# WHU-USI3DV/GAGS

Hardware: AMD Instinct MI355X
Metric: feature-raster fwd+bwd views/s (higher is better)
Workload: dtype f32

## Files before the change

### gags_amd/_lib.py

```python
import ctypes
import os
import subprocess

import torch

_HERE = os.path.dirname(os.path.abspath(__file__))
CSRC = os.path.join(_HERE, "csrc")
LIB_PATH = os.path.join(CSRC, "libgags_hip.so")

_vp, _i32, _i64, _f32, _f64 = ctypes.c_void_p, ctypes.c_int, ctypes.c_int64, ctypes.c_float, ctypes.c_double

SIGNATURES = {
    "gags_abi_version": (_i32, []),
    "gags_strerror": (ctypes.c_char_p, [_i32]),
    "gags_device_count": (_i32, []),
    "gags_project_fwd": (_i32, [_i32, _vp, _vp, _vp, _vp, _vp, _i32, _i32, _f32, _f32, _f32, _f32,
                                _vp, _vp, _vp, _vp, _vp, _vp]),
    "gags_project_fwd_raw": (_i32, [_i32, _vp, _vp, _vp, _vp, _f32, _vp, _vp, _i32, _i32, _f32, _f32, _f32, _f32,
                                    _vp, _vp, _vp, _vp, _vp, _vp, _vp, _vp, _vp, _vp]),
    "gags_project_bwd_raw": (_i32, [_i32, _vp, _vp, _vp, _vp, _f32, _vp, _vp, _i32, _i32, _f32, _vp, _vp, _vp, _vp, _vp,
                                    _vp, _vp, _vp, _vp, _vp]),
    "gags_scan_scratch_bytes": (_i64, [_i32]),
    "gags_cumsum_i32": (_i32, [_i32, _vp, _vp, _vp, _vp, _i64, _vp]),
    "gags_cumsum_gather_i32": (_i32, [_i32, _vp, _vp, _vp, _vp, _vp, _i64, _vp]),
    "gags_read_i32": (_i32, [_vp, _vp, _vp]),
    "gags_depth_order_scratch_bytes": (_i64, [_i32]),
    "gags_depth_order": (_i32, [_i32, _vp, _vp, _vp, _vp, _vp, _i64, _vp]),
    "gags_tile_emit": (_i32, [_i32, _vp, _vp, _vp, _vp, _vp, _i32, _i32, _vp, _vp, _vp]),
    "gags_tile_emit_cap": (_i32, [_i32, _vp, _vp, _vp, _vp, _vp, _i32, _i32, _vp, _vp, _i64, _vp, _vp]),
    "gags_sort_scratch_bytes": (_i64, [_i64]),
    "gags_sort_pairs": (_i32, [_i64, _i32, _i32, _vp, _vp, _vp, _vp, _vp, _i64, _vp]),
    "gags_tile_offsets": (_i32, [_i64, _vp, _i32, _vp, _vp]),
    "gags_pack_isects": (_i32, [_i32, _i64, _vp, _vp, _vp, _vp, _vp, _vp, _vp, _vp]),
    "gags_raster_fwd_scratch_bytes": (_i64, [_i64, _i32, _i32]),
    "gags_raster_fwd": (_i32, [_i32, _i32, _i32, _i32, _vp, _vp, _vp, _vp, _vp, _vp, _vp, _i64, _vp, _vp, _vp, _vp,
                               _vp, _i64, _vp, _i32, _vp]),
    "gags_raster_bwd": (_i32, [_i32, _i32, _i32, _vp, _vp, _vp, _vp, _vp, _vp, _vp, _i64, _vp, _vp, _vp, _vp, _vp,
                               _vp, _vp, _vp, _vp, _i32, _vp]),
    "gags_bwd_rowmap_scratch_bytes": (_i64, [_i64]),
    "gags_bwd_rowmap_elems": (_i64, [_i64, _i32, _i32]),
    "gags_bwd_rowmap": (_i32, [_i64, _i32, _i32, _vp, _vp, _vp, _i64, _vp, _i64, _vp, _vp, _i64, _vp]),
    "gags_raster_bwd_geom_scratch_bytes": (_i64, [_i64, _i32, _i32, _i32, _i32, _i64]),
    "gags_raster_bwd_geom": (_i32, [_i32, _i32, _i32, _i32, _vp, _vp, _vp, _i64, _vp, _vp, _vp, _vp, _vp, _i64, _vp, _i64,
                                    _vp, _vp, _vp, _i64, _i32, _vp]),
    "gags_blended_mask": (_i32, [_i64, _i32, _i32, _i32, _vp, _vp, _i64, _vp, _vp]),
    "gags_bwd_staged_scratch_bytes": (_i64, [_i64, _i32, _i32]),
    "gags_raster_bwd_colors_staged": (_i32, [_i32, _i32, _i32, _i32, _vp, _i64, _vp, _vp, _vp, _i64, _vp, _i64, _vp,
                                             _i64, _vp, _i32, _i32, _i32, _vp, _vp, _vp, _vp, _vp, _vp]),
    "gags_raster_list_need": (_i32, [_i32, _i32, _i32, _vp, _vp, _i64, _vp, _i32, _vp, _vp]),
    "gags_trim_lists": (_i32, [_i32, _i32, _vp, _vp, _vp, _vp, _vp, _vp]),
    "gags_trim_last_ids": (_i32, [_i32, _i32, _vp, _vp, _vp, _vp, _vp]),
    "gags_raster_stats": (_i32, [_i32, _i32, _vp, _vp, _vp, _vp, _vp, _i64, _vp, _vp]),
    "gags_project_bwd": (_i32, [_i32, _vp, _vp, _vp, _vp, _vp, _i32, _i32, _f32, _vp, _vp, _vp, _vp, _vp,
                                _vp, _vp, _vp, _vp]),
    "gags_sh_fwd": (_i32, [_i32, _i32, _i32, _vp, _vp, _vp, _vp, _vp, _vp]),
    "gags_sh_bwd": (_i32, [_i32, _i32, _i32, _vp, _vp, _vp, _vp, _vp, _vp, _vp]),
    "gags_sh_bwd_dirs": (_i32, [_i32, _i32, _i32, _vp, _vp, _vp, _vp, _vp, _vp, _vp, _vp]),
    "gags_ed_normalize": (_i32, [_i64, _i32, _vp, _vp, _vp]),
    "gags_adam_step": (_i32, [_i64, _vp, _vp, _vp, _vp, _f64, _f64, _f64, _f64, _i32, _vp]),
    "gags_pack_rows": (_i32, [_i64, _vp, _vp, _i32, _i32, _i32, _i32, _vp, _i32, _vp]),
    "gags_unpack_rows": (_i32, [_i64, _vp, _vp, _i32, _vp, _vp, _i32, _i32, _i32, _i32, _vp]),
    "gags_compact_mask_scratch_bytes": (_i64, [_i32]),
    "gags_compact_mask": (_i32, [_i32, _vp, _i64, _vp, _vp, _vp, _i64, _vp]),
    "gags_compact_mask_pos": (_i32, [_i32, _vp, _i64, _vp, _vp, _vp, _vp, _i64, _vp]),
    "gags_dot_scratch_bytes": (_i64, []),
    "gags_dot_f32": (_i32, [_i64, _vp, _vp, _vp, _vp, _i64, _vp]),
    "gags_trained_seg": (_i32, [_i32, _i32, _vp, _vp, _vp, _vp]),
    "gags_entropy_fwd": (_i32, [_i64, _vp, _vp, _vp]),
    "gags_entropy_bwd": (_i32, [_i64, _vp, _f32, _vp, _vp]),
    "gags_entropy_bwd_dev": (_i32, [_i64, _vp, _vp, _vp, _vp]),
    "gags_segment_stats": (_i32, [_i64, _i32, _vp, _vp, _i32, _vp, _vp, _vp, _vp]),
    "gags_segment_stats_multi": (_i32, [_i64, _i32, _vp, _vp, _i32, _i32, _vp, _vp, _vp, _i32, _vp]),
    "gags_segment_stats_runs_copies": (_i32, [_i64, _i32, _i32, _i32]),
    "gags_segment_stats_runs": (_i32, [_i64, _i32, _vp, _vp, _i32, _i32, _vp, _vp, _vp, _i32, _vp]),
    "gags_segment_loss": (_i32, [_i32, _i32, _i32, _i32, _i64, _vp, _vp, _vp, _vp, _vp, _vp, _vp, _vp, _vp, _vp]),
    "gags_region_var_bwd_layout": (_i32, [_i64, _i32, _vp, _vp, _i32, _vp, _vp, _vp, _i32, _vp]),
    "gags_region_var_bwd_add": (_i32, [_i64, _i32, _vp, _vp, _i32, _vp, _vp, _vp, _vp, _vp]),
    "gags_region_var_bwd": (_i32, [_i64, _i32, _vp, _vp, _i32, _vp, _vp, _vp, _vp]),
    "gags_gather_seg_coef": (_i32, [_i64, _vp, _i32, _vp, _vp, _vp]),
    "gags_sam_clip_feature": (_i32, [_i32, _i32, _i32, _i32, _i32, _i32, _vp, _vp, _vp, _vp, _vp, _vp]),
    "gags_sam_clip_feature_bwd_scale": (_i32, [_i32, _i32, _i32, _i32, _i32, _i32, _vp, _vp, _vp, _vp, _vp]),
    "gags_distill_l1_map_fwd": (_i32, [_i32, _i32, _i32, _i32, _i32, _i32, _vp, _vp, _vp, _vp, _vp, _vp, _i32, _vp]),
    "gags_distill_l1_map_bwd": (_i32, [_i32, _i32, _i32, _i32, _i32, _i32, _vp, _vp, _vp, _vp, _vp, _vp, _vp, _i32, _vp]),
    "gags_decoder_head_distill_fwd": (_i32, [_i32, _i32, _i32, _i32, _i32, _i32, _i32, _vp, _vp, _vp, _vp, _vp, _vp, _vp]),
    "gags_decoder_head_distill_bwd": (_i32, [_i32, _i32, _i32, _i32, _i32, _i32, _i32, _vp, _vp, _vp, _vp, _vp, _vp, _vp, _vp]),
    "gags_decoder_head_distill_bwd_f32": (_i32, [_i32, _i32, _i32, _i32, _i32, _i32, _i32, _vp, _vp, _vp, _vp, _vp, _vp, _vp, _vp]),
    "gags_decoder_pack_input": (_i32, [_i64, _i32, _i32, _vp, _vp, _vp]),
    "gags_decoder_pack_layer": (_i32, [_i32, _i32, _vp, _vp, _vp, _vp, _vp, _vp, _vp, _vp]),
    "gags_decoder_pack_layers": (_i32, [_i32, _vp, _vp, _vp, _vp, _vp, _vp, _vp, _vp, _vp, _vp]),
    "gags_decoder_layer": (_i32, [_i64, _i32, _i32, _vp, _vp, _vp, _vp, _i32, _vp, _vp, _vp, _vp, _vp, _vp]),
    "gags_decoder_wgrad_scratch_bytes": (_i64, [_i64, _i32, _i32]),
    "gags_decoder_wgrad": (_i32, [_i64, _i32, _i32, _vp, _vp, _vp, _vp, _vp, _vp, _i64, _vp]),
    "gags_decoder_wgrad_out": (_i32, [_i64, _i32, _i32, _vp, _vp, _vp, _vp, _vp, _i32, _i32, _vp, _vp, _i64, _vp]),
    "gags_decoder_head_bwd": (_i32, [_i64, _i32, _i32, _i32, _vp, _vp, _vp, _i32, _vp]),
    "gags_decoder_unpack_grad": (_i32, [_i64, _i32, _i32, _vp, _vp, _vp]),
    "gags_decoder_head": (_i32, [_i64, _i32, _i32, _i32, _vp, _vp, _i32, _vp]),
    "gags_decoder_fwd_fused": (_i32, [_i64, _i32, _i32, _vp, _vp, _vp, _vp, _vp, _vp, _vp]),
    "gags_decoder_bwd_fused": (_i32, [_i64, _i32, _i32, _vp, _vp, _vp, _vp, _vp, _vp]),
    "gags_decoder_bwd_fused_scaled": (_i32, [_i64, _i32, _i32, _vp, _vp, _vp, _vp, _vp, _vp, _vp]),
    "gags_scale_decoder_fwd_fused": (_i32, [_i64, _i32, _vp, _vp, _vp, _vp, _vp, _vp, _vp]),
    "gags_scale_decoder_fwd_fused_head": (_i32, [_i64, _i32, _vp, _vp, _vp, _vp, _vp, _vp, _vp, _vp]),
    "gags_softmax_head_bwd_y": (_i32, [_i64, _i32, _i32, _vp, _vp, _vp, _vp]),
    "gags_scale_decoder_bwd_fused": (_i32, [_i64, _vp, _vp, _vp, _vp, _vp]),
    "gags_decoder_layer_exact": (_i32, [_i64, _i32, _i32, _vp, _vp, _i32, _vp, _vp, _i32, _vp, _vp, _vp, _vp, _i32, _vp]),
    "gags_decoder_layer_split": (_i32, [_i64, _i32, _i32, _vp, _vp, _i32, _vp, _vp, _i32, _vp, _vp, _vp, _vp, _i32, _i32, _vp]),
    "gags_decoder_wgrad_split": (_i32, [_i64, _i32, _i32, _vp, _i32, _vp, _vp, _i32, _vp, _vp, _vp, _i64, _i32, _vp]),
    "gags_decoder_wgrad_exact_scratch_bytes": (_i64, [_i64, _i32, _i32]),
    "gags_decoder_wgrad_exact": (_i32, [_i64, _i32, _i32, _vp, _i32, _vp, _vp, _i32, _vp, _vp, _vp, _i64, _vp]),
    "gags_decoder_head_bwd_exact": (_i32, [_i64, _i32, _i32, _i32, _vp, _vp, _i32, _vp, _i32, _vp]),
    **{name + "_h16": None for name in ("gags_decoder_pack_layer", "gags_decoder_pack_layers", "gags_decoder_pack_input", "gags_decoder_layer", "gags_decoder_head",
                                        "gags_decoder_wgrad_scratch_bytes", "gags_decoder_wgrad", "gags_decoder_wgrad_out",
                                        "gags_decoder_head_bwd",
                                        "gags_decoder_unpack_grad", "gags_decoder_fwd_fused", "gags_decoder_bwd_fused", "gags_decoder_bwd_fused_scaled",
                                        "gags_scale_decoder_fwd_fused", "gags_scale_decoder_bwd_fused", "gags_scale_decoder_fwd_fused_head",
                                        "gags_softmax_head_bwd_y")},
    "gags_pow2_scale": (_i32, [_vp, _f32, _f32, _vp, _vp]),
    "gags_decoder_head_distill_bwd_h16": (_i32, [_i32, _i32, _i32, _i32, _i32, _i32, _i32, _vp, _vp, _vp, _vp, _vp, _vp, _vp, _vp, _vp]),
    "gags_relevancy": (_i32, [_i64, _i32, _i32, _i32, _vp, _vp, _vp, _vp, _vp]),
    "gags_relevancy_activate_scratch_bytes": (_i64, [_i32, _i32, _i32]),
    "gags_relevancy_activate": (_i32, [_i32, _i32, _i32, _vp, _f32, _i32, _i32, _vp, _vp, _vp, _vp, _vp, _vp, _vp, _i64, _vp]),
    "gags_point_relevancy_mask_scratch_bytes": (_i64, [_i32, _i64]),
    "gags_point_relevancy_mask": (_i32, [_i32, _i64, _vp, _f32, _vp, _vp, _vp, _i64, _vp]),
    "gags_point_mask_smooth_scratch_bytes": (_i64, [_i32, _i64]),
    "gags_point_mask_smooth": (_i32, [_i32, _i64, _vp, _vp, _f64, _i32, _vp, _vp, _vp, _i64, _vp]),
    "gags_depthsample_scratch_bytes": (_i64, [_i64, _i32, _i32, _i32]),
    "gags_depthsample_map": (_i32, [_i64, _i32, _i32, _i32, _vp, _vp, _vp, _vp, _f32, _i32, _vp, _vp, _vp, _vp, _i64, _vp]),
    "gags_depthsample_scatter": (_i32, [_i64, _i32, _i32, _i32, _vp, _vp, _vp, _vp, _f32, _i32, _vp, _vp, _vp, _i64, _vp]),
}

for _name in [k for k, v in SIGNATURES.items() if v is None]:
    SIGNATURES[_name] = SIGNATURES[_name[:-4]]

GAGS_BWD_COLORS_ONLY = 1
GAGS_FWD_NO_MFMA = 2
GAGS_FWD_ONLY_WEIGHTS, GAGS_FWD_ONLY_FEATURES = 512, 1024
GAGS_RECS_BY_GAUSSIAN = 256
GAGS_BWD_ATOMIC = 4
GAGS_FEAT_F16 = 32
GAGS_BWD_F32MFMA = 64
GAGS_BWD_BLOCKWAVES = 4096
GAGS_BWD_EXACT_WEIGHTS = 8192
GAGS_BWD_F16SPLIT = 0
GAGS_FWD_F16MFMA = 128
GAGS_FWD_EXACT = 2048
GAGS_FWD_FUSED = 8
GAGS_STAGE_ALL, GAGS_STAGE_ROWS, GAGS_STAGE_SORT, GAGS_STAGE_REDUCE, GAGS_STAGE_MASK = 0, 1, 2, 3, 15
GAGS_STAGED_F32MFMA, GAGS_STAGED_OUT_F16, GAGS_STAGED_PREZEROED = 32, 64, 128
GAGS_STAGED_RANGE_SCRATCH, GAGS_STAGED_BLOCKWAVES, GAGS_STAGED_EXACT_WEIGHTS = 256, 512, 1024
GAGS_GEOM_F32MFMA = 32

_lib = None


class GagsLibraryError(RuntimeError):
    pass


def build(verbose=False):
    out = None if verbose else subprocess.DEVNULL
    subprocess.check_call(["make", "-C", CSRC, "-j8", "libgags_hip.so"], stdout=out)
    return LIB_PATH


def load():
    global _lib
    if _lib is not None:
        return _lib
    if not os.path.exists(LIB_PATH):
        raise GagsLibraryError(
            f"{LIB_PATH} is missing: build it with `python -c 'import __graft_entry__ as g; g.build()'` "
            "or `make -C gags_amd/csrc`.  gags_amd has no CPU / PyTorch fallback.")
    try:
        lib = ctypes.CDLL(LIB_PATH)
    except OSError as e:
        raise GagsLibraryError(f"cannot load {LIB_PATH}: {e}") from e
    for name, (res, args) in SIGNATURES.items():
        try:
            fn = getattr(lib, name)
        except AttributeError as e:
            raise GagsLibraryError(f"{LIB_PATH} does not export {name}") from e
        fn.restype = res
        fn.argtypes = args
    _lib = lib
    return lib


def check(code, what):
    if code != 0:
        msg = load().gags_strerror(code)
        raise RuntimeError(f"{what} failed: {msg.decode() if msg else code} ({code})")


def ptr(t):
    return None if t is None else ctypes.c_void_p(t.data_ptr())
```

### gags_amd/csrc/api.hip

```cpp
#include <cstdlib>
#include "common.h"
#include "scan.h"

int gags_raster_fwd_valu(int d, int width, int height, const float *means2d, const float *conics,
                         const float *opacities, const float *colors, const float *backgrounds,
                         const int32_t *offsets, const int32_t *flat, int n_isects, float *out, float *alphas,
                         int32_t *last_ids, hipStream_t st);
int gags_raster_bwd_valu(int d, int width, int height, const float *means2d, const float *conics,
                         const float *opacities, const float *colors, const float *backgrounds,
                         const int32_t *offsets, const int32_t *flat, int n_isects, const float *alphas,
                         const int32_t *last_ids, const float *v_out, const float *v_alpha, float *v_colors,
                         float *v_opac, float *v_m2d, float *v_con, bool geom, hipStream_t st);
int gags_pack_isects_launch(int n, int n_isects, const int32_t *flat, const float *means2d, const float *conics,
                            const float *opacities, const int32_t *radii, void *grec, void *packed, hipStream_t st);
int gags_raster_weights_launch(int width, int height, int n_gauss, const void *packed, int by_gauss, const int32_t *offsets,
                               const int32_t *flat, int n_isects, float *wt, int32_t *gid_s, int32_t *sidx_s,
                               int32_t *hit, int32_t *blk_rows, float *Tbuf, float *alphas, int32_t *last_ids,
                               hipStream_t st, const float *colors16 = nullptr, const float *backgrounds = nullptr,
                               float *render_colors = nullptr);
int gags_list_need_launch(int width, int height, int n_gauss, const void *packed, int by_gauss, const int32_t *offsets,
                          const int32_t *flat, int n_isects, int32_t *need, hipStream_t st);
int gags_trim_offsets_launch(int n_tiles, const int32_t *cum, int32_t *off_new, hipStream_t st);
int gags_trim_gather_launch(int n_tiles, const int32_t *off_old, const int32_t *off_new, const int32_t *flat_in, int32_t *flat_out,
                            hipStream_t st);
int gags_trim_last_ids_launch(int width, int height, const int32_t *off_old, const int32_t *off_new, const float *alphas,
                              int32_t *last_ids, hipStream_t st);
int gags_raster_fwd_feat_launch(int d, int width, int height, int n_gauss, const float *colors, int colors_f16, int exact,
                                const float *backgrounds, const int32_t *offsets, int n_isects,
                                const int32_t *blk_rows, const float *wt, const int32_t *gid_s, const float *Tbuf,
                                float *out, hipStream_t st);
int gags_raster_fwd_fused_launch(int d, int width, int height, const void *packed, const float *colors,
                                 const float *backgrounds, const int32_t *offsets, const int32_t *flat, int n_isects,
                                 float *out, float *alphas, int32_t *last_ids, int by_gauss, hipStream_t st);
int64_t gags_bwd_staged_scratch_bytes_impl(int64_t rows, int n_gauss, int d);
int gags_raster_bwd_staged_launch(int d, int width, int height, int n_gauss, const int32_t *offsets, int n_isects,
                                  const float *v_out, const int32_t *blk_rows, const int32_t *trow, int64_t rows,
                                  const float *wt, const int32_t *gid_s, const int32_t *trow_s, void *scratch,
                                  int64_t scratch_bytes, float *v_colors, int stage, int ch_begin, int ch_count,
                                  const int32_t *rows_dev, const int32_t *wire_pos, float *wire, const uint8_t *keep_prev,
                                  uint8_t *keep_cur, hipStream_t st);
int64_t gags_raster_bwd_geom_scratch_bytes_impl(int64_t n_isects, int width, int height, int n_gauss, int d, int64_t n_rows);
int gags_raster_bwd_geom_launch(int d, int n_gauss, int width, int height, const float *colors, const float *backgrounds,
                                const int32_t *offsets, int n_isects, const void *packed, const float *v_out,
                                const float *v_alphas, const int32_t *blk_rows, const float *wt, const int32_t *gid_s,
                                const int32_t *sidx_s, const float *Tbuf, void *scratch, int64_t scratch_bytes, float *v_geo,
                                int by_gauss, const int32_t *row_base, int64_t n_rows, const int32_t *hit,
                                const int32_t *flatten_ids, int f32mfma, hipStream_t st);
int gags_blended_mask_launch(int n_isects, const int32_t *hit, const int32_t *flatten_ids, unsigned char *mask, hipStream_t st);
int gags_bwd_slot_rows_launch(int width, int height, int n_isects, const int32_t *offsets, const int32_t *blk_rows,
                              const int32_t *sidx_s, const int32_t *trow, int32_t *trow_s, hipStream_t st);
int gags_raster_bwd_atomic_launch(int d, int width, int height, const void *packed, const int32_t *offsets,
                                  const int32_t *flat, int n_isects, const float *v_out, float *v_colors,
                                  int by_gauss, hipStream_t st);

namespace {
inline int64_t al256(int64_t x) { return (x + 255) / 256 * 256; }
struct FwdScratch {
    int64_t wt, gid, sidx, hit, tbuf, total;
};
inline FwdScratch fwd_layout(int64_t n_isects, int width, int height)
{
    const int64_t tile_w = (width + GAGS_TILE - 1) / GAGS_TILE, tile_h = (height + GAGS_TILE - 1) / GAGS_TILE;
    const int64_t slots = gags_slot_count(n_isects, tile_w * tile_h);
    FwdScratch L;
    int64_t o = 0;
    L.wt = o; o += al256(slots * 256);
    L.gid = o; o += al256(slots * 4);
    L.sidx = o; o += al256(slots * 4);
    L.hit = o; o += al256((n_isects + 1) * 4);
    L.tbuf = o; o += al256((int64_t)width * height * 4);
    L.total = o;
    return L;
}
inline bool fused_width(int d) { return d >= 32 && d % 32 == 0; }
inline bool isects_ok(int64_t n_isects, int width, int height)
{
    if (n_isects < 0 || n_isects >= GAGS_MAX_ISECTS || width <= 0 || height <= 0) return false;
    const int64_t tile_w = (width + GAGS_TILE - 1) / GAGS_TILE, tile_h = (height + GAGS_TILE - 1) / GAGS_TILE;
    return gags_slot_count(n_isects, tile_w * tile_h) < (1ll << 30);
}
}

extern "C" int gags_pack_isects(int n, int64_t n_isects, const int32_t *flatten_ids, const float *means2d,
                                const float *conics, const float *opacities, const int32_t *radii, void *grec,
                                void *packed, void *stream)
{
    if (n < 0 || n_isects < 0 || n_isects >= (1ll << 31)) return GAGS_EINVAL;
    if (n_isects == 0) return GAGS_OK;
    if (!flatten_ids || !means2d || !conics || !opacities || (!packed && !grec)) return GAGS_EINVAL;
    return gags_pack_isects_launch(n, (int)n_isects, flatten_ids, means2d, conics, opacities, radii, grec, packed,
                                   (hipStream_t)stream);
}

extern "C" int64_t gags_raster_fwd_scratch_bytes(int64_t n_isects, int width, int height)
{
    if (n_isects < 0 || width <= 0 || height <= 0) return 0;
    return fwd_layout(n_isects, width, height).total;
}

namespace {
bool fwd_d16_unfused()
{
    static const bool v = [] { const char *e = getenv("GAGS_FWD_D16_UNFUSED"); return e && e[0] == '1'; }();
    return v;
}
}

extern "C" int gags_raster_fwd(int d, int n, int width, int height, const float *means2d, const float *conics,
                               const float *opacities, const float *colors, const float *backgrounds,
                               const int32_t *isect_offsets, const int32_t *flatten_ids, int64_t n_isects,
                               const void *packed, float *render_colors, float *render_alphas, int32_t *last_ids,
                               void *scratch, int64_t scratch_bytes, int32_t *blk_rows, int flags, void *stream)
{
    if (d <= 0 || n < 0 || width <= 0 || height <= 0 || !isects_ok(n_isects, width, height)) return GAGS_EINVAL;
    if (!isect_offsets || !render_colors || !render_alphas || !last_ids) return GAGS_EINVAL;
    if (n_isects > 0 && (!means2d || !conics || !opacities || !colors || !flatten_ids)) return GAGS_EINVAL;
    hipStream_t st = (hipStream_t)stream;
    const bool split = scratch && blk_rows && gags_mfma_width(d);
    if ((flags & GAGS_FEAT_F16) && (!split || (flags & GAGS_FWD_NO_MFMA) || !packed || n <= 0))
        return GAGS_EINVAL;
    if (d == 16 && !scratch && !blk_rows && packed && n > 0 && n_isects > 0 && !(flags & (GAGS_FWD_NO_MFMA | GAGS_FEAT_F16)) &&
        !(reinterpret_cast<uintptr_t>(render_colors) & 15) && !fwd_d16_unfused()) {
        return gags_raster_weights_launch(width, height, n, packed, (flags & GAGS_RECS_BY_GAUSSIAN) ? 1 : 0, isect_offsets, flatten_ids,
                                          (int)n_isects, nullptr, nullptr, nullptr, nullptr, nullptr, nullptr, render_alphas, last_ids, st,
                                          colors, backgrounds, render_colors);
    }
    if (!(flags & GAGS_FWD_NO_MFMA) && (split || fused_width(d)) && (packed || n_isects == 0) && n > 0) {
        if (split) {
            const FwdScratch L = fwd_layout(n_isects, width, height);
            if (scratch_bytes < L.total) return GAGS_ESCRATCH;
            char *sb = (char *)scratch;
            float *wt = (float *)(sb + L.wt);
            int32_t *gid_s = (int32_t *)(sb + L.gid);
            float *tbuf = (float *)(sb + L.tbuf);
            int rc = GAGS_OK;
            const bool fuse16 = d == 16 && !(flags & (GAGS_FEAT_F16 | GAGS_FWD_ONLY_FEATURES | GAGS_FWD_ONLY_WEIGHTS)) && n_isects > 0 &&
                                !(reinterpret_cast<uintptr_t>(render_colors) & 15) && !fwd_d16_unfused();
            if (!(flags & GAGS_FWD_ONLY_FEATURES))
                rc = gags_raster_weights_launch(width, height, n, packed, (flags & GAGS_RECS_BY_GAUSSIAN) ? 1 : 0, isect_offsets, flatten_ids, (int)n_isects, wt,
                                                gid_s, (int32_t *)(sb + L.sidx), (int32_t *)(sb + L.hit), blk_rows, tbuf,
                                                render_alphas, last_ids, st, fuse16 ? colors : nullptr, backgrounds, render_colors);
            if (rc != GAGS_OK || (flags & GAGS_FWD_ONLY_WEIGHTS) || fuse16) return rc;
            return gags_raster_fwd_feat_launch(d, width, height, n, colors, (flags & GAGS_FEAT_F16) ? ((flags & GAGS_FWD_F16MFMA) ? 2 : 1) : 0,
                                               (flags & GAGS_FWD_EXACT) ? 1 : 0, backgrounds, isect_offsets, (int)n_isects,
                                               blk_rows, wt, gid_s, tbuf, render_colors, st);
        }
        return gags_raster_fwd_fused_launch(d, width, height, packed, colors, backgrounds, isect_offsets, flatten_ids,
                                            (int)n_isects, render_colors, render_alphas, last_ids,
                                            (flags & GAGS_RECS_BY_GAUSSIAN) ? 1 : 0, st);
    }
    return gags_raster_fwd_valu(d, width, height, means2d, conics, opacities, colors, backgrounds, isect_offsets,
                                flatten_ids, (int)n_isects, render_colors, render_alphas, last_ids, st);
}

extern "C" int gags_raster_list_need(int n, int width, int height, const int32_t *isect_offsets, const int32_t *flatten_ids,
                                     int64_t n_isects, const void *packed, int flags, int32_t *need, void *stream)
{
    if (n < 0 || width <= 0 || height <= 0 || n_isects < 0 || n_isects >= (1ll << 31) || !need || !isect_offsets) return GAGS_EINVAL;
    if (n_isects > 0 && (!flatten_ids || !packed || n == 0)) return GAGS_EINVAL;
    return gags_list_need_launch(width, height, n, packed, (flags & GAGS_RECS_BY_GAUSSIAN) ? 1 : 0, isect_offsets, flatten_ids,
                                 (int)n_isects, need, (hipStream_t)stream);
}

extern "C" int gags_trim_lists(int width, int height, const int32_t *isect_offsets, const int32_t *need_cum,
                               const int32_t *flatten_ids, int32_t *offsets_out, int32_t *flatten_out, void *stream)
{
    if (width <= 0 || height <= 0 || !isect_offsets || !need_cum || !offsets_out) return GAGS_EINVAL;
    const int tile_w = (width + GAGS_TILE - 1) / GAGS_TILE, tile_h = (height + GAGS_TILE - 1) / GAGS_TILE;
    int rc = gags_trim_offsets_launch(tile_w * tile_h, need_cum, offsets_out, (hipStream_t)stream);
    if (rc != GAGS_OK || !flatten_out) return rc;
    if (!flatten_ids) return GAGS_EINVAL;
    return gags_trim_gather_launch(tile_w * tile_h, isect_offsets, offsets_out, flatten_ids, flatten_out, (hipStream_t)stream);
}

extern "C" int gags_trim_last_ids(int width, int height, const int32_t *isect_offsets, const int32_t *offsets_trimmed,
                                  const float *render_alphas, int32_t *last_ids, void *stream)
{
    if (width <= 0 || height <= 0 || !isect_offsets || !offsets_trimmed || !render_alphas || !last_ids) return GAGS_EINVAL;
    return gags_trim_last_ids_launch(width, height, isect_offsets, offsets_trimmed, render_alphas, last_ids, (hipStream_t)stream);
}

extern "C" int gags_raster_bwd(int d, int width, int height, const float *means2d, const float *conics,
                               const float *opacities, const float *colors, const float *backgrounds,
                               const int32_t *isect_offsets, const int32_t *flatten_ids, int64_t n_isects,
                               const void *packed, const float *render_alphas, const int32_t *last_ids,
                               const float *v_render_colors, const float *v_render_alphas, float *v_colors,
                               float *v_opacities, float *v_means2d, float *v_conics, int flags, void *stream)
{
    if (d <= 0 || width <= 0 || height <= 0 || !isects_ok(n_isects, width, height)) return GAGS_EINVAL;
    if (n_isects == 0) return GAGS_OK;
    if (!means2d || !conics || !opacities || !colors || !isect_offsets || !flatten_ids || !render_alphas ||
        !last_ids || !v_render_colors || !v_colors)
        return GAGS_EINVAL;
    const bool geom = !(flags & GAGS_BWD_COLORS_ONLY);
    if (geom && (!v_opacities || !v_means2d || !v_conics)) return GAGS_EINVAL;
    if (!geom && !(flags & GAGS_FWD_NO_MFMA) && packed) {
        const int rc = gags_raster_bwd_atomic_launch(d, width, height, packed, isect_offsets, flatten_ids,
                                                     (int)n_isects, v_render_colors, v_colors,
                                                     (flags & GAGS_RECS_BY_GAUSSIAN) ? 1 : 0, (hipStream_t)stream);
        if (rc != 1) return rc;
    }
    return gags_raster_bwd_valu(d, width, height, means2d, conics, opacities, colors, backgrounds, isect_offsets,
                                flatten_ids, (int)n_isects, render_alphas, last_ids, v_render_colors,
                                v_render_alphas, v_colors, v_opacities, v_means2d, v_conics, geom,
                                (hipStream_t)stream);
}

extern "C" int64_t gags_bwd_staged_scratch_bytes(int64_t rows, int n, int d)
{
    if (rows < 0 || n < 0 || d <= 0) return 0;
    return gags_bwd_staged_scratch_bytes_impl(rows, n, d);
}

namespace {
inline int64_t rowmap_slot_off(int64_t n_isects) { return al256((n_isects + 1) * 4) / 4; }
inline int64_t slot_count(int64_t n_isects, int width, int height)
{
    const int64_t tile_w = (width + GAGS_TILE - 1) / GAGS_TILE, tile_h = (height + GAGS_TILE - 1) / GAGS_TILE;
    return gags_slot_count(n_isects, tile_w * tile_h);
}
}

extern "C" int64_t gags_bwd_rowmap_elems(int64_t n_isects, int width, int height)
{
    if (n_isects < 0 || width <= 0 || height <= 0) return 0;
    return rowmap_slot_off(n_isects) + slot_count(n_isects, width, height);
}

extern "C" int64_t gags_bwd_rowmap_scratch_bytes(int64_t n_isects)
{
    return n_isects < 0 ? 0 : gags_scan::scratch_bytes(n_isects > 0 ? n_isects : 1);
}

extern "C" int gags_bwd_rowmap(int64_t n_isects, int width, int height, const int32_t *isect_offsets,
                               const int32_t *blk_rows, const void *fwd_scratch, int64_t fwd_scratch_bytes,
                               int32_t *rowmap, int64_t rowmap_elems, int32_t *total, void *scratch,
                               int64_t scratch_bytes, void *stream)
{
    GAGS_CLEAR_ERR();
    if (!isects_ok(n_isects, width, height) || !fwd_scratch || !rowmap || !total ||
        !isect_offsets || !blk_rows)
        return GAGS_EINVAL;
    if (rowmap_elems < gags_bwd_rowmap_elems(n_isects, width, height)) return GAGS_ESCRATCH;
    const FwdScratch L = fwd_layout(n_isects, width, height);
    if (fwd_scratch_bytes < L.total) return GAGS_ESCRATCH;
    hipStream_t st = (hipStream_t)stream;
    int32_t *trow = rowmap;
    if (hipMemsetAsync(trow, 0, sizeof(int32_t), st) != hipSuccess) return GAGS_ELAUNCH;
    if (n_isects == 0) return hipMemsetAsync(total, 0, sizeof(int32_t), st) == hipSuccess ? GAGS_OK : GAGS_ELAUNCH;
    if (!scratch || scratch_bytes < gags_scan::scratch_bytes(n_isects)) return GAGS_ESCRATCH;
    const char *fs = (const char *)fwd_scratch;
    gags_scan::launch<false>((int)n_isects, (const int32_t *)(fs + L.hit), trow + 1, total, (int32_t *)scratch, st);
    GAGS_CHECK_LAUNCH();
    return gags_bwd_slot_rows_launch(width, height, (int)n_isects, isect_offsets, blk_rows,
                                     (const int32_t *)(fs + L.sidx), trow, rowmap + rowmap_slot_off(n_isects), st);
}

extern "C" int64_t gags_raster_bwd_geom_scratch_bytes(int64_t n_isects, int width, int height, int n, int d, int64_t n_rows)
{
    if (n_isects < 0 || width <= 0 || height <= 0 || n < 0 || d <= 0) return 0;
    return gags_raster_bwd_geom_scratch_bytes_impl(n_isects, width, height, n, d, n_rows);
}

extern "C" int gags_raster_bwd_geom(int d, int n, int width, int height, const float *colors, const float *backgrounds,
                                    const int32_t *isect_offsets, int64_t n_isects, const void *packed,
                                    const float *v_render_colors, const float *v_render_alphas, const int32_t *blk_rows,
                                    const void *fwd_scratch, int64_t fwd_scratch_bytes, void *scratch, int64_t scratch_bytes,
                                    float *v_geo, const int32_t *flatten_ids, const int32_t *row_base, int64_t n_rows,
                                    int flags, void *stream)
{
    if (d <= 0 || width <= 0 || height <= 0 || n < 0 || !isects_ok(n_isects, width, height)) return GAGS_EINVAL;
    if (n == 0) return GAGS_OK;
    if (!colors || !isect_offsets || !packed || !v_render_colors || !blk_rows || !fwd_scratch || !scratch || !v_geo)
        return GAGS_EINVAL;
    const FwdScratch L = fwd_layout(n_isects, width, height);
    if (fwd_scratch_bytes < L.total) return GAGS_ESCRATCH;
    const char *fs = (const char *)fwd_scratch;
    return gags_raster_bwd_geom_launch(d, n, width, height, colors, backgrounds, isect_offsets, (int)n_isects, packed,
                                       v_render_colors, v_render_alphas, blk_rows, (const float *)(fs + L.wt),
                                       (const int32_t *)(fs + L.gid), (const int32_t *)(fs + L.sidx),
                                       (const float *)(fs + L.tbuf), scratch, scratch_bytes, v_geo,
                                       (flags & GAGS_RECS_BY_GAUSSIAN) ? 1 : 0, row_base, n_rows,
                                       (const int32_t *)(fs + L.hit), flatten_ids, (flags & GAGS_GEOM_F32MFMA) ? 1 : 0,
                                       (hipStream_t)stream);
}

extern "C" int gags_blended_mask(int64_t n_isects, int width, int height, int n, const int32_t *flatten_ids,
                                 const void *fwd_scratch, int64_t fwd_scratch_bytes, unsigned char *mask, void *stream)
{
    if (!isects_ok(n_isects, width, height) || n < 0) return GAGS_EINVAL;
    if (n == 0) return GAGS_OK;
    if (!mask) return GAGS_EINVAL;
    if (hipMemsetAsync(mask, 0, (size_t)n, (hipStream_t)stream) != hipSuccess) return GAGS_ELAUNCH;
    if (n_isects == 0) return GAGS_OK;
    if (!flatten_ids || !fwd_scratch) return GAGS_EINVAL;
    const FwdScratch L = fwd_layout(n_isects, width, height);
    if (fwd_scratch_bytes < L.total) return GAGS_ESCRATCH;
    return gags_blended_mask_launch((int)n_isects, (const int32_t *)((const char *)fwd_scratch + L.hit), flatten_ids, mask,
                                    (hipStream_t)stream);
}

extern "C" int gags_raster_bwd_colors_staged(int d, int n, int width, int height, const int32_t *isect_offsets,
                                             int64_t n_isects, const float *v_render_colors, const int32_t *blk_rows,
                                             const int32_t *rowmap, int64_t rows, const void *fwd_scratch,
                                             int64_t fwd_scratch_bytes, void *scratch, int64_t scratch_bytes,
                                             float *v_colors, int stage, int ch_begin, int ch_count,
                                             const int32_t *rows_dev, const int32_t *wire_pos, float *wire,
                                             const uint8_t *keep_prev, uint8_t *keep_cur, void *stream)
{
    if ((wire != nullptr) != (wire_pos != nullptr) || (wire && (stage & GAGS_STAGED_OUT_F16))) return GAGS_EINVAL;
    if ((keep_prev != nullptr) != (keep_cur != nullptr) || (keep_cur && (keep_prev == keep_cur || (stage & GAGS_STAGED_PREZEROED))))
        return GAGS_EINVAL;
    if (d <= 0 || width <= 0 || height <= 0 || n < 0 || !isects_ok(n_isects, width, height) || rows < 0 ||
        rows >= (1ll << 31) || stage < 0 || (stage & GAGS_STAGE_MASK) > GAGS_STAGE_REDUCE)
        return GAGS_EINVAL;
    if (n == 0) return GAGS_OK;
    if (!isect_offsets || !blk_rows || !rowmap || !fwd_scratch || !scratch || !v_colors || !v_render_colors)
        return GAGS_EINVAL;
    if (reinterpret_cast<uintptr_t>(blk_rows) & 15) return GAGS_EINVAL;
    const FwdScratch L = fwd_layout(n_isects, width, height);
    if (fwd_scratch_bytes < L.total) return GAGS_ESCRATCH;
    const char *fs = (const char *)fwd_scratch;
    return gags_raster_bwd_staged_launch(d, width, height, n, isect_offsets, (int)n_isects, v_render_colors, blk_rows,
                                         rowmap, rows, (const float *)(fs + L.wt), (const int32_t *)(fs + L.gid),
                                         rowmap + rowmap_slot_off(n_isects), scratch, scratch_bytes, v_colors, stage,
                                         ch_begin, ch_count, rows_dev, wire_pos, wire, keep_prev, keep_cur, (hipStream_t)stream);
}
```

### gags_amd/csrc/binning.hip

```cpp
#include "common.h"
#include "scan.h"

namespace {

__global__ __launch_bounds__(256) void tile_emit_kernel(int n, const float *__restrict__ means2d,
                                                        const int32_t *__restrict__ radii,
                                                        const float *__restrict__ depths,
                                                        const int32_t *__restrict__ cum,
                                                        const int32_t *__restrict__ order, int tile_w, int tile_h,
                                                        int64_t *__restrict__ isect_ids,
                                                        int32_t *__restrict__ flatten_ids, int64_t cap)
{
    __shared__ int s_rel[4][64], s_x0[4][64], s_y0[4][64], s_w[4][64], s_gid[4][64];
    __shared__ uint32_t s_dbits[4][64];
    const int lane = threadIdx.x & 63, w = threadIdx.x >> 6;
    const int j = blockIdx.x * 256 + threadIdx.x;
    const int jw = j - lane;
    if (jw >= n) return;
    const bool live = j < n;
    const int i = live ? (order ? order[j] : j) : 0;
    const int rad = live ? radii[i] : 0;
    int x0 = 0, x1 = 0, y0 = 0, y1 = 0;
    uint32_t dbits = 0;
    if (rad > 0) {
        const float2 m = reinterpret_cast<const float2 *>(means2d)[i];
        gags_tile_aabb(m.x, m.y, rad, tile_w, tile_h, x0, x1, y0, y1);
        dbits = (uint32_t)__float_as_int(depths[i]);
    }
    const int base = (jw == 0) ? 0 : cum[jw - 1];
    const int start = live ? ((j == 0) ? 0 : cum[j - 1]) : 0x7fffffff;
    const int jl = min(jw + 63, n - 1);
    const int total = cum[jl] - base;
    s_rel[w][lane] = live ? start - base : 0x7fffffff;
    s_x0[w][lane] = x0; s_y0[w][lane] = y0; s_w[w][lane] = max(x1 - x0, 1); s_gid[w][lane] = i; s_dbits[w][lane] = dbits;
    __builtin_amdgcn_wave_barrier();
    for (int t = lane; t < total; t += 64) {
        int l = 0;
#pragma unroll
        for (int step = 32; step > 0; step >>= 1)
            if (s_rel[w][l + step] <= t) l += step;
        const int r = t - s_rel[w][l];
        const int ww = s_w[w][l];
        const int dy = r / ww;
        const int64_t tile_id = (int64_t)(s_y0[w][l] + dy) * tile_w + (s_x0[w][l] + (r - dy * ww));
        const int64_t pos = (int64_t)base + t;
        if (pos < cap) {
            isect_ids[pos] = (tile_id << 32) | (int64_t)s_dbits[w][l];
            flatten_ids[pos] = s_gid[w][l];
        }
    }
}

__global__ __launch_bounds__(256) void isect_tail_kernel(int64_t cap, const int32_t *__restrict__ total, int n_tiles,
                                                         int64_t *__restrict__ isect_ids, int32_t *__restrict__ flatten_ids)
{
    const int64_t i = (int64_t)blockIdx.x * 256 + threadIdx.x;
    if (i >= cap || i < (int64_t)total[0]) return;
    isect_ids[i] = (int64_t)n_tiles << 32;
    flatten_ids[i] = 0;
}

__global__ __launch_bounds__(256) void tile_offsets_kernel(int64_t n_isects, const int64_t *__restrict__ sorted_ids,
                                                           int n_tiles, int32_t *__restrict__ offsets)
{
    const int64_t idx = (int64_t)blockIdx.x * 256 + threadIdx.x;
    if (idx >= n_isects) return;
    const int cur = (int)((uint64_t)sorted_ids[idx] >> 32);
    if (idx == 0) {
        for (int t = 0; t <= cur; ++t) offsets[t] = 0;
    } else {
        const int prev = (int)((uint64_t)sorted_ids[idx - 1] >> 32);
        for (int t = prev + 1; t <= cur; ++t) offsets[t] = (int32_t)idx;
    }
    if (idx == n_isects - 1)
        for (int t = cur + 1; t < n_tiles; ++t) offsets[t] = (int32_t)n_isects;
}

__global__ void fill_i32_kernel(int n, int32_t v, int32_t *__restrict__ out)
{
    const int i = blockIdx.x * 256 + threadIdx.x;
    if (i < n) out[i] = v;
}

__global__ __launch_bounds__(256) void ed_normalize_kernel(int64_t n_pix, int d, float *__restrict__ colors,
                                                           const float *__restrict__ alphas)
{
    const int64_t i = (int64_t)blockIdx.x * 256 + threadIdx.x;
    if (i >= n_pix) return;
    colors[i * d + (d - 1)] = colors[i * d + (d - 1)] / fmaxf(alphas[i], 1e-10f);
}

}

extern "C" int gags_abi_version(void) { return 2; }

extern "C" const char *gags_strerror(int code)
{
    switch (code) {
        case GAGS_OK: return "ok";
        case GAGS_EINVAL: return "invalid argument";
        case GAGS_ELAUNCH: return "HIP launch/runtime error";
        case GAGS_ESCRATCH: return "scratch buffer too small";
        case GAGS_ENODEV: return "no usable gfx950 device";
        default: return "unknown error";
    }
}

extern "C" int gags_device_count(void)
{
    GAGS_CLEAR_ERR();
    int n = 0;
    if (hipGetDeviceCount(&n) != hipSuccess) return GAGS_ENODEV;
    return n;
}

extern "C" int64_t gags_scan_scratch_bytes(int n)
{
    return gags_scan::scratch_bytes(n);
}

extern "C" int gags_cumsum_i32(int n, const int32_t *in, int32_t *cum, int32_t *total, void *scratch,
                               int64_t scratch_bytes, void *stream)
{
    GAGS_CLEAR_ERR();
    if (n < 0) return GAGS_EINVAL;
    hipStream_t st = (hipStream_t)stream;
    if (n == 0) {
        if (total) hipLaunchKernelGGL(fill_i32_kernel, dim3(1), dim3(256), 0, st, 1, 0, total);
        GAGS_CHECK_LAUNCH();
        return GAGS_OK;
    }
    if (!in || !cum || !scratch) return GAGS_EINVAL;
    if (scratch_bytes < gags_scan_scratch_bytes(n)) return GAGS_ESCRATCH;
    gags_scan::launch<false>(n, in, cum, total, (int32_t *)scratch, st);
    GAGS_CHECK_LAUNCH();
    return GAGS_OK;
}

extern "C" int gags_cumsum_gather_i32(int n, const int32_t *in, const int32_t *idx, int32_t *cum, int32_t *total, void *scratch,
                                      int64_t scratch_bytes, void *stream)
{
    GAGS_CLEAR_ERR();
    if (n < 0) return GAGS_EINVAL;
    hipStream_t st = (hipStream_t)stream;
    if (n == 0) {
        if (total) hipLaunchKernelGGL(fill_i32_kernel, dim3(1), dim3(256), 0, st, 1, 0, total);
        GAGS_CHECK_LAUNCH();
        return GAGS_OK;
    }
    if (!in || !idx || !cum || !scratch || in == cum) return GAGS_EINVAL;
    if (scratch_bytes < gags_scan_scratch_bytes(n)) return GAGS_ESCRATCH;
    gags_scan::launch<false>(n, in, cum, total, (int32_t *)scratch, st, idx);
    GAGS_CHECK_LAUNCH();
    return GAGS_OK;
}

extern "C" int gags_read_i32(const int32_t *src, int32_t *dst_host, void *stream)
{
    GAGS_CLEAR_ERR();
    if (!src || !dst_host) return GAGS_EINVAL;
    if (hipMemcpyAsync(dst_host, src, sizeof(int32_t), hipMemcpyDeviceToHost, (hipStream_t)stream) != hipSuccess)
        return GAGS_ELAUNCH;
    if (hipStreamSynchronize((hipStream_t)stream) != hipSuccess) return GAGS_ELAUNCH;
    return GAGS_OK;
}

extern "C" int gags_tile_emit_cap(int n, const float *means2d, const int32_t *radii, const float *depths, const int32_t *cum,
                                  const int32_t *order, int tile_w, int tile_h, int64_t *isect_ids, int32_t *flatten_ids,
                                  int64_t cap, const int32_t *total, void *stream)
{
    GAGS_CLEAR_ERR();
    if (n < 0 || tile_w <= 0 || tile_h <= 0 || cap < 0 || cap >= (1ll << 31)) return GAGS_EINVAL;
    if (n == 0 && cap == 0) return GAGS_OK;
    if (!isect_ids || !flatten_ids || (n > 0 && (!means2d || !radii || !depths || !cum))) return GAGS_EINVAL;
    hipStream_t st = (hipStream_t)stream;
    if (n > 0)
        hipLaunchKernelGGL(tile_emit_kernel, dim3((n + 255) / 256), dim3(256), 0, st, n, means2d, radii, depths, cum, order, tile_w,
                           tile_h, isect_ids, flatten_ids, cap);
    if (total && cap > 0)
        hipLaunchKernelGGL(isect_tail_kernel, dim3((unsigned)((cap + 255) / 256)), dim3(256), 0, st, cap, total, tile_w * tile_h,
                           isect_ids, flatten_ids);
    GAGS_CHECK_LAUNCH();
    return GAGS_OK;
}

extern "C" int gags_tile_emit(int n, const float *means2d, const int32_t *radii, const float *depths,
                              const int32_t *cum, const int32_t *order, int tile_w, int tile_h, int64_t *isect_ids,
                              int32_t *flatten_ids, void *stream)
{
    if (n == 0) return GAGS_OK;
    return gags_tile_emit_cap(n, means2d, radii, depths, cum, order, tile_w, tile_h, isect_ids, flatten_ids, (1ll << 31) - 1, nullptr,
                              stream);
}

extern "C" int gags_tile_offsets(int64_t n_isects, const int64_t *sorted_ids, int n_tiles, int32_t *isect_offsets,
                                 void *stream)
{
    GAGS_CLEAR_ERR();
    if (n_isects < 0 || n_tiles <= 0 || !isect_offsets) return GAGS_EINVAL;
    hipStream_t st = (hipStream_t)stream;
    if (n_isects == 0) {
        hipLaunchKernelGGL(fill_i32_kernel, dim3((n_tiles + 1 + 255) / 256), dim3(256), 0, st, n_tiles + 1, 0, isect_offsets);
        GAGS_CHECK_LAUNCH();
        return GAGS_OK;
    }
    if (!sorted_ids) return GAGS_EINVAL;
    hipLaunchKernelGGL(tile_offsets_kernel, dim3((unsigned)((n_isects + 255) / 256)), dim3(256), 0, st, n_isects,
                       sorted_ids, n_tiles + 1, isect_offsets);
    GAGS_CHECK_LAUNCH();
    return GAGS_OK;
}

extern "C" int gags_ed_normalize(int64_t n_pix, int d, float *render_colors, const float *render_alphas,
                                 void *stream)
{
    GAGS_CLEAR_ERR();
    if (n_pix < 0 || d <= 0) return GAGS_EINVAL;
    if (n_pix == 0) return GAGS_OK;
    if (!render_colors || !render_alphas) return GAGS_EINVAL;
    hipLaunchKernelGGL(ed_normalize_kernel, dim3((unsigned)((n_pix + 255) / 256)), dim3(256), 0,
                       (hipStream_t)stream, n_pix, d, render_colors, render_alphas);
    GAGS_CHECK_LAUNCH();
    return GAGS_OK;
}
```

### gags_amd/csrc/exchange.hip

```cpp
#include <hip/hip_bf16.h>
#include <hip/hip_fp16.h>
#include "common.h"
#include "scan.h"

namespace {

template <int T> struct Elem;
template <> struct Elem<0> {
    using type = float;
    static __device__ __forceinline__ float ld(const void *p, size_t i) { return reinterpret_cast<const float *>(p)[i]; }
    static __device__ __forceinline__ void st(void *p, size_t i, float v) { reinterpret_cast<float *>(p)[i] = v; }
    static __device__ __forceinline__ float4 ld4(const void *p, size_t i) { return *reinterpret_cast<const float4 *>(reinterpret_cast<const float *>(p) + i); }
    static __device__ __forceinline__ void st4(void *p, size_t i, float4 v) { *reinterpret_cast<float4 *>(reinterpret_cast<float *>(p) + i) = v; }
};
template <> struct Elem<1> {
    using type = __half;
    static __device__ __forceinline__ float ld(const void *p, size_t i) { return __half2float(reinterpret_cast<const __half *>(p)[i]); }
    static __device__ __forceinline__ void st(void *p, size_t i, float v) { reinterpret_cast<__half *>(p)[i] = __float2half_rn(v); }
    static __device__ __forceinline__ float4 ld4(const void *p, size_t i)
    {
        const uint2 u = *reinterpret_cast<const uint2 *>(reinterpret_cast<const __half *>(p) + i);
        const __half2 a = *reinterpret_cast<const __half2 *>(&u.x), b = *reinterpret_cast<const __half2 *>(&u.y);
        return make_float4(__low2float(a), __high2float(a), __low2float(b), __high2float(b));
    }
    static __device__ __forceinline__ void st4(void *p, size_t i, float4 v)
    {
        const __half2 a = __floats2half2_rn(v.x, v.y), b = __floats2half2_rn(v.z, v.w);
        uint2 u;
        u.x = *reinterpret_cast<const unsigned *>(&a); u.y = *reinterpret_cast<const unsigned *>(&b);
        *reinterpret_cast<uint2 *>(reinterpret_cast<__half *>(p) + i) = u;
    }
};
template <> struct Elem<2> {
    using type = __hip_bfloat16;
    static __device__ __forceinline__ float ld(const void *p, size_t i) { return __bfloat162float(reinterpret_cast<const __hip_bfloat16 *>(p)[i]); }
    static __device__ __forceinline__ void st(void *p, size_t i, float v) { reinterpret_cast<__hip_bfloat16 *>(p)[i] = __float2bfloat16(v); }
    static __device__ __forceinline__ float4 ld4(const void *p, size_t i)
    {
        const uint2 u = *reinterpret_cast<const uint2 *>(reinterpret_cast<const __hip_bfloat16 *>(p) + i);
        return make_float4(__uint_as_float(u.x << 16), __uint_as_float(u.x & 0xffff0000u), __uint_as_float(u.y << 16),
                           __uint_as_float(u.y & 0xffff0000u));
    }
    static __device__ __forceinline__ void st4(void *p, size_t i, float4 v)
    {
        __hip_bfloat16 h[4] = {__float2bfloat16(v.x), __float2bfloat16(v.y), __float2bfloat16(v.z), __float2bfloat16(v.w)};
        *reinterpret_cast<uint2 *>(reinterpret_cast<__hip_bfloat16 *>(p) + i) = *reinterpret_cast<const uint2 *>(h);
    }
};

template <int TG, int TW, bool V4>
__global__ __launch_bounds__(256) void pack_rows_kernel(int64_t n_rows, const int64_t *__restrict__ idx,
                                                        const void *__restrict__ grad, int d, int c0, int cw,
                                                        void *__restrict__ wire)
{
    const int q = (cw + 3) >> 2;
    const int64_t t = (int64_t)blockIdx.x * 256 + threadIdx.x;
    if (t >= n_rows * q) return;
    const int64_t r = t / q;
    const int c = (int)(t - r * q) * 4;
    const int64_t gi = idx ? idx[r] : r;
    const bool pad = gi < 0;
    const int64_t g = pad ? 0 : gi;
    if constexpr (V4) {
        float4 v = Elem<TG>::ld4(grad, (size_t)g * d + c0 + c);
        if (pad) v = make_float4(0.f, 0.f, 0.f, 0.f);
        Elem<TW>::st4(wire, (size_t)r * cw + c, v);
    } else {
        float v[4];
#pragma unroll
        for (int e = 0; e < 4; ++e) {
            v[e] = Elem<TG>::ld(grad, (size_t)g * d + c0 + min(c + e, cw - 1));
            if (pad) v[e] = 0.f;
        }
#pragma unroll
        for (int e = 0; e < 4; ++e) asm volatile("" : "+v"(v[e]));
#pragma unroll
        for (int e = 0; e < 4; ++e)
            if (c + e < cw) Elem<TW>::st(wire, (size_t)r * cw + c + e, v[e]);
    }
}

template <int TG, int TW, bool DELTA, bool V4>
__global__ __launch_bounds__(256) void unpack_rows_kernel(int64_t n_rows, const int64_t *__restrict__ idx,
                                                          const void *__restrict__ wire, const void *__restrict__ local,
                                                          void *__restrict__ grad, int d, int c0, int cw)
{
    const int q = (cw + 3) >> 2;
    const int64_t t = (int64_t)blockIdx.x * 256 + threadIdx.x;
    if (t >= n_rows * q) return;
    const int64_t r = t / q;
    const int c = (int)(t - r * q) * 4;
    const int64_t g = idx ? idx[r] : r;
    if (g < 0) return;
    if constexpr (V4) {
        const size_t wi = (size_t)r * cw + c, gi = (size_t)g * d + c0 + c;
        float4 v = Elem<TW>::ld4(wire, wi);
        if constexpr (DELTA) {
            const float4 o = Elem<TG>::ld4(grad, gi), l = Elem<TW>::ld4(local, wi);
            v = make_float4(o.x + (v.x - l.x), o.y + (v.y - l.y), o.z + (v.z - l.z), o.w + (v.w - l.w));
        }
        Elem<TG>::st4(grad, gi, v);
    } else {
        float v[4];
#pragma unroll
        for (int e = 0; e < 4; ++e) {
            const size_t wi = (size_t)r * cw + min(c + e, cw - 1), gi = (size_t)g * d + c0 + min(c + e, cw - 1);
            v[e] = Elem<TW>::ld(wire, wi);
            if constexpr (DELTA) v[e] = Elem<TG>::ld(grad, gi) + (v[e] - Elem<TW>::ld(local, wi));
        }
#pragma unroll
        for (int e = 0; e < 4; ++e) asm volatile("" : "+v"(v[e]));
#pragma unroll
        for (int e = 0; e < 4; ++e)
            if (c + e < cw) Elem<TG>::st(grad, (size_t)g * d + c0 + c + e, v[e]);
    }
}

constexpr int CM_PER_THREAD = 8, CM_TILE = 256 * CM_PER_THREAD;

__device__ __forceinline__ int cm_load(const uint8_t *__restrict__ mask, int n, int base, unsigned &bits)
{
    bits = 0;
#pragma unroll
    for (int e = 0; e < CM_PER_THREAD; ++e)
        if (base + e < n && mask[base + e]) bits |= 1u << e;
    return __popc(bits);
}

__global__ __launch_bounds__(256) void cm_count_kernel(int n, const uint8_t *__restrict__ mask, int32_t *__restrict__ block_sums)
{
    __shared__ int smem[4];
    unsigned bits;
    const int c = cm_load(mask, n, blockIdx.x * CM_TILE + threadIdx.x * CM_PER_THREAD, bits);
    int total;
    gags_scan::block_incl_scan(c, total, smem);
    if (threadIdx.x == 0) block_sums[blockIdx.x] = total;
}

__global__ __launch_bounds__(256) void cm_scatter_kernel(int n, const uint8_t *__restrict__ mask, const int32_t *__restrict__ block_offs,
                                                         const int32_t *__restrict__ total, int64_t cap, int64_t *__restrict__ idx,
                                                         int32_t *__restrict__ inv)
{
    __shared__ int smem[4];
    unsigned bits;
    const int base = blockIdx.x * CM_TILE + threadIdx.x * CM_PER_THREAD;
    const int c = cm_load(mask, n, base, bits);
    int tot;
    const int incl = gags_scan::block_incl_scan(c, tot, smem);
    int64_t pos = (int64_t)block_offs[blockIdx.x] + incl - c;
#pragma unroll
    for (int e = 0; e < CM_PER_THREAD; ++e) {
        const bool set = (bits & (1u << e)) != 0;
        if (set && pos < cap) idx[pos] = base + e;
        if (inv && base + e < n) inv[base + e] = (set && pos < cap) ? (int32_t)pos : -1;
        if (set) ++pos;
    }
    const int64_t cnt = total[0];
    for (int64_t i = (int64_t)blockIdx.x * 256 + threadIdx.x; i < cap; i += (int64_t)gridDim.x * 256)
        if (i >= cnt) idx[i] = -1;
}

inline bool aligned16(const void *p) { return (reinterpret_cast<uintptr_t>(p) & 15) == 0; }

inline bool ok_types(int tg, int tw) { return (tg == 0 || tg == 1) && (tw == 0 || tw == 1 || tw == 2); }

}

extern "C" int gags_pack_rows(int64_t n_rows, const int64_t *idx, const void *grad, int grad_type, int d, int c0, int cw,
                              void *wire, int wire_type, void *stream)
{
    if (n_rows < 0 || d <= 0 || c0 < 0 || cw <= 0 || c0 + cw > d || !ok_types(grad_type, wire_type)) return GAGS_EINVAL;
    if (n_rows == 0) return GAGS_OK;
    if (!grad || !wire) return GAGS_EINVAL;
    GAGS_CLEAR_ERR();
    const int64_t items = n_rows * ((cw + 3) >> 2);
    const dim3 grid((unsigned)((items + 255) / 256));
    hipStream_t st = (hipStream_t)stream;
    const bool v4 = ((d | c0 | cw) & 3) == 0 && aligned16(grad) && aligned16(wire);
#define GO(TG, TW)                                                                                                         \
    do {                                                                                                                   \
        if (v4) hipLaunchKernelGGL((pack_rows_kernel<TG, TW, true>), grid, dim3(256), 0, st, n_rows, idx, grad, d, c0, cw, wire); \
        else hipLaunchKernelGGL((pack_rows_kernel<TG, TW, false>), grid, dim3(256), 0, st, n_rows, idx, grad, d, c0, cw, wire);  \
    } while (0)
    if (grad_type == 0) { if (wire_type == 0) GO(0, 0); else if (wire_type == 1) GO(0, 1); else GO(0, 2); }
    else { if (wire_type == 0) GO(1, 0); else if (wire_type == 1) GO(1, 1); else GO(1, 2); }
#undef GO
    GAGS_CHECK_LAUNCH();
    return GAGS_OK;
}

extern "C" int gags_unpack_rows(int64_t n_rows, const int64_t *idx, const void *wire, int wire_type, const void *local,
                                void *grad, int grad_type, int d, int c0, int cw, void *stream)
{
    if (n_rows < 0 || d <= 0 || c0 < 0 || cw <= 0 || c0 + cw > d || !ok_types(grad_type, wire_type)) return GAGS_EINVAL;
    if (n_rows == 0) return GAGS_OK;
    if (!grad || !wire) return GAGS_EINVAL;
    GAGS_CLEAR_ERR();
    const int64_t items = n_rows * ((cw + 3) >> 2);
    const dim3 grid((unsigned)((items + 255) / 256));
    hipStream_t st = (hipStream_t)stream;
    const bool v4 = ((d | c0 | cw) & 3) == 0 && aligned16(grad) && aligned16(wire) && (!local || aligned16(local));
#define GO1(TG, TW, V)                                                                                                     \
    do {                                                                                                                   \
        if (local) hipLaunchKernelGGL((unpack_rows_kernel<TG, TW, true, V>), grid, dim3(256), 0, st, n_rows, idx, wire, local, grad, d, c0, cw); \
        else hipLaunchKernelGGL((unpack_rows_kernel<TG, TW, false, V>), grid, dim3(256), 0, st, n_rows, idx, wire, local, grad, d, c0, cw);      \
    } while (0)
#define GO(TG, TW)                                                                                                         \
    do {                                                                                                                   \
        if (v4) GO1(TG, TW, true); else GO1(TG, TW, false);                                                                \
    } while (0)
    if (grad_type == 0) { if (wire_type == 0) GO(0, 0); else if (wire_type == 1) GO(0, 1); else GO(0, 2); }
    else { if (wire_type == 0) GO(1, 0); else if (wire_type == 1) GO(1, 1); else GO(1, 2); }
#undef GO
#undef GO1
    GAGS_CHECK_LAUNCH();
    return GAGS_OK;
}

extern "C" int64_t gags_compact_mask_scratch_bytes(int n)
{
    const int64_t nb = ((int64_t)(n > 0 ? n : 0) + CM_TILE - 1) / CM_TILE;
    return (nb > 0 ? nb : 1) * (int64_t)sizeof(int32_t);
}

extern "C" int gags_compact_mask(int n, const uint8_t *mask, int64_t cap, int64_t *idx, int32_t *count, void *scratch,
                                 int64_t scratch_bytes, void *stream)
{
    return gags_compact_mask_pos(n, mask, cap, idx, nullptr, count, scratch, scratch_bytes, stream);
}

extern "C" int gags_compact_mask_pos(int n, const uint8_t *mask, int64_t cap, int64_t *idx, int32_t *pos, int32_t *count,
                                     void *scratch, int64_t scratch_bytes, void *stream)
{
    if (n < 0 || cap < 0 || cap >= (1ll << 31) || !count || (cap > 0 && !idx)) return GAGS_EINVAL;
    hipStream_t st = (hipStream_t)stream;
    GAGS_CLEAR_ERR();
    if (n == 0) {
        (void)hipMemsetAsync(count, 0, sizeof(int32_t), st);
        if (cap > 0) (void)hipMemsetAsync(idx, 0xff, (size_t)cap * sizeof(int64_t), st);
        GAGS_CHECK_LAUNCH();
        return GAGS_OK;
    }
    if (!mask || !scratch) return GAGS_EINVAL;
    if (scratch_bytes < gags_compact_mask_scratch_bytes(n)) return GAGS_ESCRATCH;
    const int nb = (n + CM_TILE - 1) / CM_TILE;
    int32_t *bs = (int32_t *)scratch;
    hipLaunchKernelGGL(cm_count_kernel, dim3(nb), dim3(256), 0, st, n, mask, bs);
    hipLaunchKernelGGL(gags_scan::scan_spine, dim3(1), dim3(gags_scan::SCAN_THREADS), 0, st, nb, bs, count);
    hipLaunchKernelGGL(cm_scatter_kernel, dim3(nb), dim3(256), 0, st, n, mask, bs, count, cap, idx, pos);
    GAGS_CHECK_LAUNCH();
    return GAGS_OK;
}
```

### gags_amd/csrc/scan.h

```cpp
#pragma once
#include "common.h"

namespace gags_scan {
namespace {

constexpr int SCAN_THREADS = 256;
constexpr int SCAN_ITEMS = 8;
constexpr int SCAN_TILE = SCAN_THREADS * SCAN_ITEMS;

__device__ __forceinline__ int wave_incl_scan(int v)
{
    const int lane = threadIdx.x & 63;
#pragma unroll
    for (int d = 1; d < 64; d <<= 1) {
        const int o = __shfl_up(v, d, 64);
        if (lane >= d) v += o;
    }
    return v;
}

__device__ __forceinline__ int block_incl_scan(int v, int &total, int *smem )
{
    const int lane = threadIdx.x & 63, w = threadIdx.x >> 6;
    const int s = wave_incl_scan(v);
    if (lane == 63) smem[w] = s;
    __syncthreads();
    int off = 0;
#pragma unroll
    for (int k = 0; k < 4; ++k) {
        const int t = smem[k];
        if (k < w) off += t;
    }
    total = smem[0] + smem[1] + smem[2] + smem[3];
    __syncthreads();
    return s + off;
}

__global__ __launch_bounds__(SCAN_THREADS) void scan_block_sums(int n, const int32_t *__restrict__ in,
                                                                 const int32_t *__restrict__ idx,
                                                                 int32_t *__restrict__ block_sums)
{
    __shared__ int smem[4];
    const int base = blockIdx.x * SCAN_TILE;
    int s = 0;
#pragma unroll
    for (int k = 0; k < SCAN_ITEMS; ++k) {
        const int i = base + k * SCAN_THREADS + threadIdx.x;
        s += (i < n) ? in[idx ? idx[i] : i] : 0;
    }
    int total;
    block_incl_scan(s, total, smem);
    if (threadIdx.x == 0) block_sums[blockIdx.x] = total;
}

__global__ __launch_bounds__(SCAN_THREADS) void scan_spine(int nb, int32_t *__restrict__ block_sums,
                                                           int32_t *__restrict__ total_out)
{
    __shared__ int smem[4];
    __shared__ double wide[SCAN_THREADS];
    int carry = 0;
    double dsum = 0.0;
    for (int base = 0; base < nb; base += SCAN_THREADS) {
        const int i = base + threadIdx.x;
        const int v = (i < nb) ? block_sums[i] : 0;
        dsum += (double)v;
        int total;
        const int incl = block_incl_scan(v, total, smem);
        if (i < nb) block_sums[i] = carry + incl - v;
        carry += total;
    }
    wide[threadIdx.x] = dsum;
    __syncthreads();
    if (threadIdx.x == 0 && total_out) {
        double t = 0.0;
        for (int k = 0; k < SCAN_THREADS; ++k) t += wide[k];
        total_out[0] = (t > 2147483647.0) ? -1 : carry;
    }
}

template <bool EXCLUSIVE>
__global__ __launch_bounds__(SCAN_THREADS) void scan_final(int n, const int32_t *in ,
                                                            const int32_t *__restrict__ idx,
                                                            const int32_t *__restrict__ block_offs,
                                                            int32_t *out)
{
    __shared__ int smem[4];
    const int base = blockIdx.x * SCAN_TILE + threadIdx.x * SCAN_ITEMS;
    int v[SCAN_ITEMS];
    int s = 0;
#pragma unroll
    for (int k = 0; k < SCAN_ITEMS; ++k) {
        const int i = base + k;
        v[k] = (i < n) ? in[idx ? idx[i] : i] : 0;
        s += v[k];
    }
    int total;
    const int incl = block_incl_scan(s, total, smem);
    int run = block_offs[blockIdx.x] + incl - s;
#pragma unroll
    for (int k = 0; k < SCAN_ITEMS; ++k) {
        const int i = base + k;
        if (EXCLUSIVE) {
            if (i < n) out[i] = run;
            run += v[k];
        } else {
            run += v[k];
            if (i < n) out[i] = run;
        }
    }
}


}

inline int64_t scratch_bytes(int64_t n)
{
    const int64_t nb = (n + SCAN_TILE - 1) / SCAN_TILE;
    return (nb > 0 ? nb : 1) * (int64_t)sizeof(int32_t);
}

template <bool EXCLUSIVE>
inline void launch(int n, const int32_t *in, int32_t *out, int32_t *total, int32_t *block_scratch, hipStream_t st,
                   const int32_t *idx = nullptr)
{
    const int nb = (n + SCAN_TILE - 1) / SCAN_TILE;
    hipLaunchKernelGGL(scan_block_sums, dim3(nb), dim3(SCAN_THREADS), 0, st, n, in, idx, block_scratch);
    hipLaunchKernelGGL(scan_spine, dim3(1), dim3(SCAN_THREADS), 0, st, nb, block_scratch, total);
    hipLaunchKernelGGL(scan_final<EXCLUSIVE>, dim3(nb), dim3(SCAN_THREADS), 0, st, n, in, idx, block_scratch, out);
}

}
```

### gags_amd/csrc/sort.hip

```cpp
#include "common.h"
#include "scan.h"

namespace {

constexpr int RS_THREADS = 256;
constexpr int RS_ITEMS = 8;
constexpr int RS_TILE = RS_THREADS * RS_ITEMS;
constexpr int RS_RADIX = 256;

template <typename K>
__global__ __launch_bounds__(RS_THREADS) void rs_histogram(int64_t n, int shift, const K *__restrict__ keys,
                                                           uint32_t *__restrict__ hist ,
                                                           int nblocks)
{
    __shared__ uint32_t h[RS_RADIX];
    h[threadIdx.x] = 0;
    __syncthreads();
    const int64_t base = (int64_t)blockIdx.x * RS_TILE;
#pragma unroll
    for (int k = 0; k < RS_ITEMS; ++k) {
        const int64_t i = base + k * RS_THREADS + threadIdx.x;
        if (i < n) atomicAdd(&h[(keys[i] >> shift) & 0xff], 1u);
    }
    __syncthreads();
    hist[(size_t)threadIdx.x * nblocks + blockIdx.x] = h[threadIdx.x];
}

__global__ __launch_bounds__(RS_THREADS) void rs_rowscan(int nblocks, uint32_t *__restrict__ hist, uint32_t *__restrict__ totals)
{
    __shared__ int smem[4];
    uint32_t *row = hist + (size_t)blockIdx.x * nblocks;
    uint32_t carry = 0;
    for (int base = 0; base < nblocks; base += RS_TILE) {
        const int i0 = base + threadIdx.x * RS_ITEMS;
        uint32_t v[RS_ITEMS];
        uint32_t s = 0;
#pragma unroll
        for (int k = 0; k < RS_ITEMS; ++k) {
            v[k] = (i0 + k < nblocks) ? row[i0 + k] : 0u;
            s += v[k];
        }
        int total;
        const int incl = gags_scan::block_incl_scan((int)s, total, smem);
        uint32_t run = carry + (uint32_t)incl - s;
#pragma unroll
        for (int k = 0; k < RS_ITEMS; ++k) {
            if (i0 + k < nblocks) row[i0 + k] = run;
            run += v[k];
        }
        carry += (uint32_t)total;
    }
    if (threadIdx.x == 0) totals[blockIdx.x] = carry;
}

template <typename K>
__global__ __launch_bounds__(RS_THREADS) void rs_scatter(int64_t n, int shift, const K *__restrict__ keys_in,
                                                         const int32_t *__restrict__ vals_in,
                                                         K *__restrict__ keys_out,
                                                         int32_t *__restrict__ vals_out,
                                                         const uint32_t *__restrict__ hist, int nblocks,
                                                         const uint32_t *__restrict__ totals)
{
    __shared__ uint32_t cnt_s[4][RS_RADIX];
    volatile uint32_t(*cnt)[RS_RADIX] = cnt_s;
    __shared__ uint32_t gbase[RS_RADIX];
    __shared__ int scan_tmp[4];
    const int lane = threadIdx.x & 63, w = threadIdx.x >> 6;
#pragma unroll
    for (int k = 0; k < 4; ++k) cnt[k][threadIdx.x] = 0;
    {
        const uint32_t tot = totals[threadIdx.x];
        int all;
        const int incl = gags_scan::block_incl_scan((int)tot, all, scan_tmp);
        gbase[threadIdx.x] = ((uint32_t)incl - tot) + hist[(size_t)threadIdx.x * nblocks + blockIdx.x];
    }
    __syncthreads();

    const int64_t wbase = (int64_t)blockIdx.x * RS_TILE + (int64_t)w * (64 * RS_ITEMS);
    K key[RS_ITEMS];
    int32_t val[RS_ITEMS];
    uint32_t rank[RS_ITEMS];
#pragma unroll
    for (int k = 0; k < RS_ITEMS; ++k) {
        const int64_t i = wbase + k * 64 + lane;
        const bool ok = i < n;
        key[k] = ok ? keys_in[i] : (K)~(K)0;
        val[k] = ok ? (vals_in ? vals_in[i] : (int32_t)i) : 0;
        const uint32_t dgt = ok ? (uint32_t)((key[k] >> shift) & 0xff) : 0xffffffffu;
        uint64_t m = __ballot(ok);
#pragma unroll
        for (int b = 0; b < 8; ++b) {
            const uint64_t bal = __ballot((dgt >> b) & 1u);
            m &= ((dgt >> b) & 1u) ? bal : ~bal;
        }
        const uint64_t lower = m & ((1ull << lane) - 1ull);
        const uint32_t before = (uint32_t)__popcll(lower);
        uint32_t prev = 0;
        if (ok) {
            prev = cnt[w][dgt];
        }
        __builtin_amdgcn_wave_barrier();
        if (ok && lower == 0) cnt[w][dgt] = prev + (uint32_t)__popcll(m);
        __builtin_amdgcn_wave_barrier();
        rank[k] = prev + before;
    }
    __syncthreads();
    __shared__ uint32_t dstart[RS_RADIX];
    {
        const int d = threadIdx.x;
        uint32_t run = 0;
#pragma unroll
        for (int k = 0; k < 4; ++k) {
            const uint32_t c = cnt[k][d];
            cnt[k][d] = run;
            run += c;
        }
        int total;
        const int incl = gags_scan::block_incl_scan((int)run, total, scan_tmp);
        dstart[d] = (uint32_t)incl - run;
    }
    __syncthreads();
    __shared__ K keys_l[RS_TILE];
    __shared__ int32_t vals_l[RS_TILE];
#pragma unroll
    for (int k = 0; k < RS_ITEMS; ++k) {
        const int64_t i = wbase + k * 64 + lane;
        if (i < n) {
            const uint32_t dgt = (uint32_t)((key[k] >> shift) & 0xff);
            const uint32_t lp = dstart[dgt] + cnt[w][dgt] + rank[k];
            keys_l[lp] = key[k];
            vals_l[lp] = val[k];
        }
    }
    __syncthreads();
    const int64_t bbase = (int64_t)blockIdx.x * RS_TILE;
    const int nvalid = (int)((n - bbase) < (int64_t)RS_TILE ? (n - bbase) : (int64_t)RS_TILE);
#pragma unroll
    for (int k = 0; k < RS_ITEMS; ++k) {
        const int i = k * RS_THREADS + threadIdx.x;
        if (i < nvalid) {
            const K kk = keys_l[i];
            const uint32_t dgt = (uint32_t)((kk >> shift) & 0xff);
            const uint32_t pos = gbase[dgt] + ((uint32_t)i - dstart[dgt]);
            keys_out[pos] = kk;
            vals_out[pos] = vals_l[i];
        }
    }
}

template <typename K>
int64_t sort_scratch_bytes_t(int64_t n_in)
{
    const int64_t n = n_in > 0 ? n_in : 1;
    const int64_t nblocks = (n + RS_TILE - 1) / RS_TILE;
    const int64_t keys = ((n * (int64_t)sizeof(K) + 255) / 256) * 256, vals = ((n * 4 + 255) / 256) * 256;
    const int64_t hist = ((nblocks * RS_RADIX * 4 + 255) / 256) * 256;
    return keys + vals + hist + RS_RADIX * 4;
}

template <typename K>
int sort_pairs_t(int64_t n, int first_bit, int nbits, const K *keys_in, const int32_t *vals_in, K *keys_out,
                 int32_t *vals_out, void *scratch, int64_t scratch_bytes, hipStream_t st)
{
    if (n == 0) return GAGS_OK;
    if (n < 0 || n >= (1ll << 31) || nbits <= 0 || first_bit < 0 || first_bit + nbits > (int)(8 * sizeof(K)))
        return GAGS_EINVAL;
    if (!keys_in || !keys_out || !vals_out || !scratch) return GAGS_EINVAL;
    if (scratch_bytes < sort_scratch_bytes_t<K>(n)) return GAGS_ESCRATCH;
    const int nblocks = (int)((n + RS_TILE - 1) / RS_TILE);
    const int64_t keys_b = ((n * (int64_t)sizeof(K) + 255) / 256) * 256, vals_b = ((n * 4 + 255) / 256) * 256;
    K *ktmp = (K *)scratch;
    int32_t *vtmp = (int32_t *)((char *)scratch + keys_b);
    uint32_t *hist = (uint32_t *)((char *)scratch + keys_b + vals_b);
    const int64_t hist_b = (((int64_t)nblocks * RS_RADIX * 4 + 255) / 256) * 256;
    uint32_t *totals = (uint32_t *)((char *)scratch + keys_b + vals_b + hist_b);
    const int passes = (nbits + 7) / 8;
    const K *src_k = keys_in;
    const int32_t *src_v = vals_in;
    for (int p = 0; p < passes; ++p) {
        const bool to_out = ((passes - 1 - p) % 2) == 0;
        K *dst_k = to_out ? keys_out : ktmp;
        int32_t *dst_v = to_out ? vals_out : vtmp;
        hipLaunchKernelGGL(rs_histogram<K>, dim3(nblocks), dim3(RS_THREADS), 0, st, n, first_bit + p * 8, src_k, hist, nblocks);
        hipLaunchKernelGGL(rs_rowscan, dim3(RS_RADIX), dim3(RS_THREADS), 0, st, nblocks, hist, totals);
        hipLaunchKernelGGL(rs_scatter<K>, dim3(nblocks), dim3(RS_THREADS), 0, st, n, first_bit + p * 8, src_k, src_v, dst_k, dst_v,
                           hist, nblocks, totals);
        src_k = dst_k;
        src_v = dst_v;
    }
    GAGS_CHECK_LAUNCH();
    return GAGS_OK;
}

}

int64_t gags_sort_u32_scratch_bytes(int64_t n) { return sort_scratch_bytes_t<uint32_t>(n); }
int gags_sort_pairs_u32(int64_t n, int nbits, const uint32_t *keys_in, const int32_t *vals_in, uint32_t *keys_out,
                        int32_t *vals_out, void *scratch, int64_t scratch_bytes, hipStream_t st)
{
    GAGS_CLEAR_ERR();
    return sort_pairs_t<uint32_t>(n, 0, nbits, keys_in, vals_in, keys_out, vals_out, scratch, scratch_bytes, st);
}

int64_t gags_sort_u64_scratch_bytes(int64_t n) { return sort_scratch_bytes_t<uint64_t>(n); }
int gags_sort_pairs_u64(int64_t n, int first_bit, int nbits, const uint64_t *keys_in, const int32_t *vals_in,
                        uint64_t *keys_out, int32_t *vals_out, void *scratch, int64_t scratch_bytes, hipStream_t st)
{
    return sort_pairs_t<uint64_t>(n, first_bit, nbits, keys_in, vals_in, keys_out, vals_out, scratch, scratch_bytes, st);
}

extern "C" int64_t gags_sort_scratch_bytes(int64_t n_isects) { return sort_scratch_bytes_t<uint64_t>(n_isects); }

extern "C" int gags_sort_pairs(int64_t n, int tile_bits, int depth_sorted, const int64_t *keys_in,
                               const int32_t *vals_in, int64_t *keys_out, int32_t *vals_out, void *scratch,
                               int64_t scratch_bytes, void *stream)
{
    GAGS_CLEAR_ERR();
    if (n < 0 || tile_bits < 0 || tile_bits > 31) return GAGS_EINVAL;
    const int first = depth_sorted ? 32 : 0, nbits = depth_sorted ? (tile_bits > 0 ? tile_bits : 1) : 32 + tile_bits;
    return sort_pairs_t<uint64_t>(n, first, nbits, (const uint64_t *)keys_in, vals_in, (uint64_t *)keys_out, vals_out,
                                  scratch, scratch_bytes, (hipStream_t)stream);
}

namespace {
__global__ __launch_bounds__(256) void gather_i32_kernel(int n, const int32_t *__restrict__ idx,
                                                         const int32_t *__restrict__ src, int32_t *__restrict__ dst)
{
    const int i = blockIdx.x * 256 + threadIdx.x;
    if (i < n) dst[i] = src[idx[i]];
}
inline int64_t al256s(int64_t x) { return (x + 255) / 256 * 256; }
}

extern "C" int64_t gags_depth_order_scratch_bytes(int n)
{
    const int64_t m = n > 0 ? n : 1;
    return 2 * al256s(m * 4) + sort_scratch_bytes_t<uint32_t>(m);
}

extern "C" int gags_depth_order(int n, const float *depths, const int32_t *tiles_per_gauss, int32_t *order,
                                int32_t *tiles_ordered, void *scratch, int64_t scratch_bytes, void *stream)
{
    GAGS_CLEAR_ERR();
    if (n < 0) return GAGS_EINVAL;
    if (n == 0) return GAGS_OK;
    if (!depths || !order || !scratch || (tiles_ordered && !tiles_per_gauss)) return GAGS_EINVAL;
    if (scratch_bytes < gags_depth_order_scratch_bytes(n)) return GAGS_ESCRATCH;
    hipStream_t st = (hipStream_t)stream;
    char *sb = (char *)scratch;
    uint32_t *keys_sorted = (uint32_t *)(sb + al256s((int64_t)n * 4));
    void *sort_scratch = sb + 2 * al256s((int64_t)n * 4);
    const int rc = sort_pairs_t<uint32_t>(n, 0, 32, reinterpret_cast<const uint32_t *>(depths), nullptr, keys_sorted, order,
                                          sort_scratch, sort_scratch_bytes_t<uint32_t>(n), st);
    if (rc != GAGS_OK) return rc;
    if (tiles_ordered)
        hipLaunchKernelGGL(gather_i32_kernel, dim3((n + 255) / 256), dim3(256), 0, st, n, order, tiles_per_gauss,
                           tiles_ordered);
    GAGS_CHECK_LAUNCH();
    return GAGS_OK;
}
```

### gags_amd/rasterization.py

```python
import ctypes
import os
import threading
from typing import Any, NamedTuple

import torch

from . import _lib, profiler
from ._lib import check, ptr

TILE = 16
MAX_ISECTS = 1 << 28
ZERO_FILL_MIN_ELEMS = 1 << 24
GEOM_COMPACT_ROWS = True
CAP_MARGIN = 1.05
GRAD_RANGE_CHANNELS = 128
GRAD_ROWS_GROUP = 128
PROW_MAX_BYTES = 24 << 30
TRIM_LISTS = {"1": True, "0": False}.get(os.environ.get("GAGS_TRIM_LISTS", ""), None)
TRIM_AUTO_BYTES = 48 << 30
KEEP_GRAD = os.environ.get("GAGS_KEEP_GRAD", "1") != "0"
KEEP_GRAD_MIN_ELEMS = 0
KEEP_GRAD_SHAPES = 2
EARLY_COUNT = os.environ.get("GAGS_EARLY_COUNT", "1") != "0"
EARLY_ROWMAP = os.environ.get("GAGS_EARLY_ROWMAP", "1") != "0"
CAPACITY_MODE = os.environ.get("GAGS_CAPACITY_MODE", "0") == "1"


def _tiles(width, height):
    tile_w, tile_h = (width + TILE - 1) // TILE, (height + TILE - 1) // TILE
    return tile_w, tile_h, tile_w * tile_h


def _dev_key(dev):
    return dev.index if dev.index is not None else torch.cuda.current_device()


class RasterContext:

    def __init__(self, capacity_mode=None, overlap_zero_fill=False):
        self.grad_range_hook = None
        self.grad_rows_hook = None
        self.grad_wire_hook = None
        self.grad_range_channels = GRAD_RANGE_CHANNELS
        self.grad_rows_group = GRAD_ROWS_GROUP
        self.capacity_mode = CAPACITY_MODE if capacity_mode is None else bool(capacity_mode)
        self.cap_isects = {}
        self.cap_rows = {}
        self.overlap_zero_fill = bool(overlap_zero_fill)
        self.early_rowmap = EARLY_ROWMAP
        self._pinned_pool = {}
        self.k_cache = {}
        self._pinned = {}
        self._side = {}
        self.trim_lists = TRIM_LISTS
        self.keep_grad_buffer = KEEP_GRAD
        self._kept = {}
        self._kept_fails = {}

    def forget_kept(self, n, d, dtype, dev):
        self._kept.pop((n, d, dtype, dev.index), None)

    def forget_all_kept(self):
        self._kept.clear()

    def kept_grad(self, n, d, dtype, dev):
        if not self.keep_grad_buffer or not _CAN_COUNT_REFS or n * d < KEEP_GRAD_MIN_ELEMS or n == 0:
            return None
        key = (n, d, dtype, dev.index)
        if self._kept_fails.get(key, 0) >= 3:
            return None
        ent = self._kept.pop(key, None)
        if ent is not None and ent.released() and not ent.untouched():
            ent.wipe()
        if ent is not None and not ent.untouched():
            self._kept_fails[key] = self._kept_fails.get(key, 0) + 1
            ent = None
            if self._kept_fails[key] >= 3:
                return None
        elif ent is not None:
            self._kept_fails[key] = 0
        if ent is None:
            ent = _KeptGrad(n, d, dtype, dev)
        self._kept[key] = ent
        while len(self._kept) > KEEP_GRAD_SHAPES:
            self._kept.pop(next(iter(self._kept)))
        return ent.hand_out()

    def side_stream(self, dev):
        key = _dev_key(dev)
        if key not in self._side:
            self._side[key] = torch.cuda.Stream(device=dev)
        return self._side[key]

    def take_pinned(self, dev):
        key = _dev_key(dev)
        pool = self._pinned_pool.setdefault(key, [])
        return pool.pop() if pool else torch.empty(1, dtype=torch.int32).pin_memory()

    def give_pinned(self, dev, t):
        key = _dev_key(dev)
        pool = self._pinned_pool.setdefault(key, [])
        if len(pool) < 8:
            pool.append(t)

    def pinned_i64(self, dev):
        key = ("i64", _dev_key(dev))
        if key not in self._pinned:
            self._pinned[key] = torch.empty(1, dtype=torch.int64).pin_memory()
        return self._pinned[key]

    def pinned_i32(self, dev):
        key = _dev_key(dev)
        if key not in self._pinned:
            self._pinned[key] = torch.empty(1, dtype=torch.int32).pin_memory()
        return self._pinned[key]


def grad_written(grad):
    torch.autograd.graph.increment_version(grad)
    return grad


_TLS = threading.local()


def default_context():
    ctx = getattr(_TLS, "ctx", None)
    if ctx is None:
        ctx = _TLS.ctx = RasterContext()
    return ctx


def _storage_refs(t):
    return torch._C._storage_Use_Count(t.untyped_storage()._cdata)


_CAN_COUNT_REFS = hasattr(torch._C, "_storage_Use_Count")


class _KeptGrad:

    def __init__(self, n, d, dtype, dev):
        self.buf = torch.zeros(n, d, dtype=dtype, device=dev)
        self.flags = torch.zeros(2, max(n, 1), dtype=torch.uint8, device=dev)
        self.cur = 0
        self.base = _storage_refs(self.buf)
        self.version = self.buf._version

    def released(self):
        return _storage_refs(self.buf) <= self.base

    def untouched(self):
        return self.released() and self.buf._version == self.version

    def wipe(self):
        self.buf.zero_()
        self.flags.zero_()
        self.version = self.buf._version

    def hand_out(self):
        prev, cur = self.flags[self.cur], self.flags[1 - self.cur]
        self.cur ^= 1
        return self.buf.detach(), prev, cur


class _DeferredCount:

    def __init__(self, scalar, rctx):
        self.t = scalar
        self.rctx = rctx
        self.ev = torch.cuda.Event()
        self.ev.record()

    def get(self):
        dev = self.t.device
        side = self.rctx.side_stream(dev)
        host = self.rctx.pinned_i32(dev)
        done = torch.cuda.Event()
        with torch.cuda.stream(side):
            side.wait_event(self.ev)
            host.copy_(self.t, non_blocking=True)
            done.record()
        self.t.record_stream(side)
        done.synchronize()
        return int(host[0])


def _stream():
    return ctypes.c_void_p(torch.cuda.current_stream().cuda_stream)


def _need_cuda(*ts):
    cur = None
    for t in ts:
        if t is None:
            continue
        if not t.is_cuda:
            raise RuntimeError("gags_amd.rasterization: all tensors must live on the GPU "
                               "(there is no CPU path; see oracle/ for the test-only CPU restatement)")
        if cur is None:
            cur = torch.cuda.current_device()
        if t.device.index != cur:
            raise RuntimeError(f"gags_amd.rasterization: tensor on cuda:{t.device.index} but the current device is "
                               f"cuda:{cur}; one process per GPU, torch.cuda.set_device(local_rank) first")


def _c(t):
    return t if (t.is_contiguous() and t.dtype == torch.float32) else t.contiguous().float()


class _Project(torch.autograd.Function):

    @staticmethod
    def forward(ctx, means, quats, scales, viewmat, K, width, height, eps2d, near, far, radius_clip):
        lib = _lib.load()
        means, quats, scales, viewmat, K = _c(means), _c(quats), _c(scales), _c(viewmat), _c(K)
        n = means.shape[0]
        dev = means.device
        radii = torch.empty(n, dtype=torch.int32, device=dev)
        means2d = torch.empty(n, 2, dtype=torch.float32, device=dev)
        depths = torch.empty(n, dtype=torch.float32, device=dev)
        conics = torch.empty(n, 3, dtype=torch.float32, device=dev)
        tiles = torch.empty(n, dtype=torch.int32, device=dev)
        with profiler.stage("project_fwd"):
            check(lib.gags_project_fwd(n, ptr(means), ptr(quats), ptr(scales), ptr(viewmat), ptr(K), width, height,
                                       eps2d, near, far, radius_clip, ptr(radii), ptr(means2d), ptr(depths),
                                       ptr(conics), ptr(tiles), _stream()), "gags_project_fwd")
        ctx.save_for_backward(means, quats, scales, viewmat, K, radii, conics)
        ctx.cfg = (width, height, eps2d)
        ctx.mark_non_differentiable(radii, tiles)
        return radii, means2d, depths, conics, tiles

    @staticmethod
    def backward(ctx, _v_radii, v_means2d, v_depths, v_conics, _v_tiles):
        lib = _lib.load()
        means, quats, scales, viewmat, K, radii, conics = ctx.saved_tensors
        width, height, eps2d = ctx.cfg
        n = means.shape[0]
        dev = means.device
        v_means2d = torch.zeros(n, 2, device=dev) if v_means2d is None else _c(v_means2d)
        v_conics = torch.zeros(n, 3, device=dev) if v_conics is None else _c(v_conics)
        v_depths = None if v_depths is None else _c(v_depths)
        v_means = torch.empty(n, 3, device=dev)
        v_quats = torch.empty(n, 4, device=dev)
        v_scales = torch.empty(n, 3, device=dev)
        check(lib.gags_project_bwd(n, ptr(means), ptr(quats), ptr(scales), ptr(viewmat), ptr(K), width, height,
                                   eps2d, ptr(radii), ptr(conics), ptr(v_means2d), ptr(v_depths), ptr(v_conics),
                                   ptr(v_means), ptr(v_quats), ptr(v_scales), _stream()), "gags_project_bwd")
        return v_means, v_quats, v_scales, None, None, None, None, None, None, None, None


class _ProjectRaw(torch.autograd.Function):

    @staticmethod
    def forward(ctx, means, rotation, scaling_log, opacity_logit, viewmat, K, width, height, eps2d, near, far, radius_clip,
                scaling_modifier, want_records):
        lib = _lib.load()
        means, rotation, scaling_log, viewmat, K = _c(means), _c(rotation), _c(scaling_log), _c(viewmat), _c(K)
        logit = _c(opacity_logit.reshape(-1))
        n = means.shape[0]
        dev = means.device
        radii = torch.empty(n, dtype=torch.int32, device=dev)
        means2d = torch.empty(n, 2, dtype=torch.float32, device=dev)
        depths = torch.empty(n, dtype=torch.float32, device=dev)
        conics = torch.empty(n, 3, dtype=torch.float32, device=dev)
        tiles = torch.empty(n, dtype=torch.int32, device=dev)
        opac = torch.empty(n, dtype=torch.float32, device=dev)
        grec = torch.empty(max(n, 1), 8, dtype=torch.float32, device=dev) if want_records else torch.empty(0, device=dev)
        with profiler.stage("project_fwd"):
            check(lib.gags_project_fwd_raw(n, ptr(means), ptr(rotation), ptr(scaling_log), ptr(logit), scaling_modifier,
                                           ptr(viewmat), ptr(K), width, height, eps2d, near, far, radius_clip, ptr(radii),
                                           ptr(means2d), ptr(depths), ptr(conics), ptr(tiles), ptr(opac), None, None,
                                           ptr(grec) if want_records else None, _stream()), "gags_project_fwd_raw")
        ctx.save_for_backward(means, rotation, scaling_log, logit, viewmat, K, radii)
        ctx.cfg = (width, height, eps2d, scaling_modifier, tuple(opacity_logit.shape))
        ctx.mark_non_differentiable(radii, tiles, grec)
        return radii, means2d, depths, conics, tiles, opac, grec

    @staticmethod
    def backward(ctx, _v_radii, v_means2d, v_depths, v_conics, _v_tiles, v_opac, _v_grec):
        lib = _lib.load()
        means, rotation, scaling_log, logit, viewmat, K, radii = ctx.saved_tensors
        width, height, eps2d, modifier, oshape = ctx.cfg
        n = means.shape[0]
        dev = means.device
        v_means2d = torch.zeros(n, 2, device=dev) if v_means2d is None else _c(v_means2d)
        v_conics = torch.zeros(n, 3, device=dev) if v_conics is None else _c(v_conics)
        v_depths = None if v_depths is None else _c(v_depths)
        v_opac = None if v_opac is None else _c(v_opac)
        v_means = torch.empty(n, 3, device=dev)
        v_rot = torch.empty(n, 4, device=dev)
        v_scal = torch.empty(n, 3, device=dev)
        v_logit = torch.empty(n, device=dev) if ctx.needs_input_grad[3] else None
        check(lib.gags_project_bwd_raw(n, ptr(means), ptr(rotation), ptr(scaling_log), ptr(logit), modifier, ptr(viewmat),
                                       ptr(K), width, height, eps2d, ptr(radii), ptr(v_means2d), ptr(v_depths),
                                       ptr(v_conics), ptr(v_opac), ptr(v_means), ptr(v_rot), ptr(v_scal), ptr(v_logit),
                                       _stream()), "gags_project_bwd_raw")
        return (v_means, v_rot, v_scal, None if v_logit is None else v_logit.reshape(oshape), None, None, None, None, None,
                None, None, None, None, None)


class _SH(torch.autograd.Function):

    @staticmethod
    def forward(ctx, coeffs, means, campos, radii, degree):
        lib = _lib.load()
        coeffs, means, campos = _c(coeffs), _c(means), _c(campos)
        n, kc = coeffs.shape[0], coeffs.shape[1]
        out = torch.empty(n, 3, device=coeffs.device)
        check(lib.gags_sh_fwd(n, kc, degree, ptr(means), ptr(campos), ptr(coeffs), ptr(radii), ptr(out), _stream()),
              "gags_sh_fwd")
        ctx.save_for_backward(means, campos, radii, out, coeffs if ctx.needs_input_grad[1] else None)
        ctx.cfg = (kc, degree)
        return out

    @staticmethod
    def backward(ctx, v_out):
        lib = _lib.load()
        means, campos, radii, out, coeffs = ctx.saved_tensors
        kc, degree = ctx.cfg
        n = means.shape[0]
        v_out = _c(v_out)
        v_coeffs = v_means = None
        if ctx.needs_input_grad[0]:
            v_coeffs = torch.empty(n, kc, 3, device=means.device)
            check(lib.gags_sh_bwd(n, kc, degree, ptr(means), ptr(campos), ptr(radii), ptr(out), ptr(v_out),
                                  ptr(v_coeffs), _stream()), "gags_sh_bwd")
        if ctx.needs_input_grad[1]:
            v_means = torch.empty(n, 3, device=means.device)
            check(lib.gags_sh_bwd_dirs(n, kc, degree, ptr(means), ptr(campos), ptr(coeffs), ptr(radii), ptr(out),
                                       ptr(v_out), ptr(v_means), _stream()), "gags_sh_bwd_dirs")
        return v_coeffs, v_means, None, None, None


class Binning(NamedTuple):
    isect_ids: Any
    flatten_ids: Any
    isect_offsets: Any
    n_isects: Any
    packed: Any
    offsets_full: Any


def tile_binning(means2d, radii, depths, tiles_per_gauss, width, height, conics=None, opacities=None, cap=None, records=None,
                 context=None):
    lib = _lib.load()
    st = _stream()
    dev = means2d.device
    n = radii.shape[0]
    tile_w, tile_h, n_tiles = _tiles(width, height)
    tile_bits = max(1, n_tiles.bit_length())
    cum = torch.empty(max(n, 1), dtype=torch.int32, device=dev)
    total = torch.empty(1, dtype=torch.int32, device=dev)
    early = None
    if cap is None and EARLY_COUNT and n > 0:
        host64 = (context or default_context()).pinned_i64(dev)
        host64.copy_(tiles_per_gauss.sum().reshape(1), non_blocking=True)
        early = torch.cuda.Event()
        early.record()
    order = torch.empty(max(n, 1), dtype=torch.int32, device=dev)
    dsb = lib.gags_depth_order_scratch_bytes(n)
    dscratch = torch.empty(dsb, dtype=torch.uint8, device=dev)
    check(lib.gags_depth_order(n, ptr(depths), None, ptr(order), None, ptr(dscratch), dsb, st), "gags_depth_order")
    sb = lib.gags_scan_scratch_bytes(n)
    scratch = torch.empty(sb, dtype=torch.uint8, device=dev)
    check(lib.gags_cumsum_gather_i32(n, ptr(tiles_per_gauss), ptr(order), ptr(cum), ptr(total), ptr(scratch), sb, st),
          "gags_cumsum_gather_i32")
    if cap is None:
        if early is not None:
            early.synchronize()
            n_isects = int(host64[0])
        else:
            host = ctypes.c_int32(0)
            check(lib.gags_read_i32(ptr(total), ctypes.byref(host), st), "gags_read_i32")
            n_isects = int(host.value)
        _check_isects(n_isects, n_tiles)
        size, count = n_isects, n_isects
    else:
        size, count = int(cap), _DeferredCount(total, context or default_context())
    offsets = torch.empty(n_tiles + 1, dtype=torch.int32, device=dev)
    ids = torch.empty(max(size, 1), dtype=torch.int64, device=dev)
    flat = torch.empty(max(size, 1), dtype=torch.int32, device=dev)
    ids_s = torch.empty_like(ids)
    flat_s = torch.empty_like(flat)
    if size > 0:
        check(lib.gags_tile_emit_cap(n, ptr(means2d), ptr(radii), ptr(depths), ptr(cum), ptr(order), tile_w, tile_h,
                                     ptr(ids), ptr(flat), size, ptr(total) if cap is not None else None, st),
              "gags_tile_emit_cap")
        ssb = lib.gags_sort_scratch_bytes(size)
        sscratch = torch.empty(ssb, dtype=torch.uint8, device=dev)
        check(lib.gags_sort_pairs(size, tile_bits, 1, ptr(ids), ptr(flat), ptr(ids_s), ptr(flat_s), ptr(sscratch),
                                  ssb, st), "gags_sort_pairs")
    check(lib.gags_tile_offsets(size, ptr(ids_s), n_tiles, ptr(offsets), st), "gags_tile_offsets")
    packed = records
    if conics is not None and packed is None:
        packed = torch.empty(max(n, 1), 8, dtype=torch.float32, device=dev)
        check(lib.gags_pack_isects(n, size, ptr(flat_s), ptr(means2d), ptr(conics), ptr(opacities), ptr(radii),
                                   ptr(packed), None, st), "gags_pack_isects")
    off_view = offsets[:n_tiles].view(tile_h, tile_w)
    return Binning(ids_s[:size], flat_s[:size], off_view, count, packed, offsets)


def _trim_lists(lib, n, width, height, offsets_full, flatten_ids, n_isects, packed):
    st = _stream()
    dev = flatten_ids.device
    n_tiles = _tiles(width, height)[2]
    need = torch.empty(n_tiles, dtype=torch.int32, device=dev)
    with profiler.stage("list_need"):
        check(lib.gags_raster_list_need(n, width, height, ptr(offsets_full), ptr(flatten_ids), n_isects, ptr(packed),
                                        _lib.GAGS_RECS_BY_GAUSSIAN, ptr(need), st), "gags_raster_list_need")
    cum = torch.empty(n_tiles, dtype=torch.int32, device=dev)
    total = torch.empty(1, dtype=torch.int32, device=dev)
    sb = lib.gags_scan_scratch_bytes(n_tiles)
    scratch = torch.empty(sb, dtype=torch.uint8, device=dev)
    check(lib.gags_cumsum_i32(n_tiles, ptr(need), ptr(cum), ptr(total), ptr(scratch), sb, st), "gags_cumsum_i32")
    host = ctypes.c_int32(0)
    check(lib.gags_read_i32(ptr(total), ctypes.byref(host), st), "gags_read_i32")
    t = int(host.value)
    offs_t = torch.empty(n_tiles + 1, dtype=torch.int32, device=dev)
    flat_t = torch.empty(t, dtype=torch.int32, device=dev)
    check(lib.gags_trim_lists(width, height, ptr(offsets_full), ptr(cum), ptr(flatten_ids), ptr(offs_t),
                              ptr(flat_t) if t > 0 else None, st), "gags_trim_lists")
    return offs_t, flat_t, t


def _check_isects(n_isects, n_tiles=0):
    if n_isects < 0 or n_isects >= MAX_ISECTS or 4 * n_isects + 64 * n_tiles + 64 >= (1 << 30):
        raise RuntimeError(f"gags_amd.rasterization: {n_isects if n_isects >= 0 else '> 2^31'} tile intersections in one "
                           f"view; the kernels index at most 2^28 = {MAX_ISECTS} less 16 per tile (INTEGRATION.md, memory model)")


def _mfma_width(d):
    return d >= 16


class _Rasterize(torch.autograd.Function):

    @staticmethod
    def forward(ctx, means2d, conics, colors, opacities, backgrounds, offsets, flatten_ids, packed, width, height,
                flags, prezero=None, rctx=None, n_isects=None, grad_on=True):
        lib = _lib.load()
        needs = tuple(bool(g) and bool(grad_on) for g in ctx.needs_input_grad)
        means2d, conics, opacities = _c(means2d), _c(conics), _c(opacities)
        half = (colors.dtype == torch.float16 and packed is not None and colors.shape[0] > 0
                and not (flags & (_lib.GAGS_FWD_NO_MFMA | _lib.GAGS_FWD_FUSED)))
        colors = (colors if colors.is_contiguous() else colors.contiguous()) if half else _c(colors)
        backgrounds = None if backgrounds is None else _c(backgrounds)
        n, d = colors.shape
        dev = colors.device
        n_tiles = _tiles(width, height)[2]
        offsets = _offsets_with_count(offsets, n_tiles, flatten_ids.shape[0] if n_isects is None else n_isects)
        n_isects = flatten_ids.shape[0]
        out = torch.empty(height, width, d, device=dev)
        alphas = torch.empty(height, width, device=dev)
        last_ids = torch.empty(height, width, dtype=torch.int32, device=dev)
        split = n > 0 and packed is not None and not (flags & (_lib.GAGS_FWD_NO_MFMA | _lib.GAGS_FWD_FUSED))
        scratch = blk_rows = None
        nbytes = 0
        lean16 = (split and d == 16 and not half and n_isects > 0 and not any(needs)
                  and not (flags & _lib.GAGS_FWD_EXACT) and not profiler.ENABLED)
        if split and not lean16:
            nbytes = lib.gags_raster_fwd_scratch_bytes(n_isects, width, height)
            try:
                scratch = torch.empty(nbytes, dtype=torch.uint8, device=dev)
            except torch.OutOfMemoryError:
                (rctx if rctx is not None else default_context()).forget_all_kept()
                try:
                    scratch = torch.empty(nbytes, dtype=torch.uint8, device=dev)
                except torch.OutOfMemoryError:
                    scratch = None
            if scratch is None:
                import warnings
                warnings.warn(f"gags_amd.rasterization: {nbytes / 2 ** 30:.1f} GiB of forward scratch for {n_isects} tile "
                              "intersections could not be allocated; this view runs on the scratch-free kernels "
                              "(INTEGRATION.md, memory model)", RuntimeWarning, stacklevel=3)
                split, nbytes, scratch = False, 0, None
                if half:
                    half, colors = False, colors.float()
        if lean16:
            split = False
        if split:
            blk_rows = torch.empty(n_tiles * 4, dtype=torch.int32, device=dev)
        cflags = ((flags & 3) | (flags & _lib.GAGS_FWD_EXACT) | _lib.GAGS_RECS_BY_GAUSSIAN | (_lib.GAGS_FEAT_F16 if half else 0)
                  | (64 if (half and d >= 128 and (flags & _lib.GAGS_FWD_F16MFMA)) else 0))

        def launch(extra=0):
            check(lib.gags_raster_fwd(d, n, width, height, ptr(means2d), ptr(conics), ptr(opacities), ptr(colors),
                                      ptr(backgrounds), ptr(offsets), ptr(flatten_ids), n_isects, ptr(packed),
                                      ptr(out), ptr(alphas), ptr(last_ids), ptr(scratch), nbytes, ptr(blk_rows),
                                      cflags | extra, _stream()), "gags_raster_fwd")

        with profiler.stage("raster_fwd"):
            if profiler.ENABLED and split and n_isects > 0:
                with profiler.stage("raster_weights"):
                    launch(_lib.GAGS_FWD_ONLY_WEIGHTS)
                with profiler.stage("raster_fwd_feat"):
                    launch(_lib.GAGS_FWD_ONLY_FEATURES)
            else:
                launch()
        if split:
            profiler.note("fwd_blk_rows", blk_rows)
        need_geom = needs[0] or needs[1] or needs[3]
        rctx_ = rctx if rctx is not None else default_context()
        early = None
        if (split and n_isects > 0 and rctx_.early_rowmap and needs[2] and not need_geom and _mfma_width(d)
                and d <= 1024 and not (flags & _lib.GAGS_BWD_ATOMIC) and not rctx_.capacity_mode):
            with profiler.stage("bwd_rowcount"):
                early = _early_rowmap(lib, rctx_, _FwdState(offsets, n_isects, blk_rows, scratch, flatten_ids, n, d, width, height))
        geom_mfma = split and need_geom and _geom_mfma_width(d) and not (flags & _lib.GAGS_BWD_ATOMIC)
        staged = (split and _mfma_width(d) and d <= 1024 and (needs[2] or geom_mfma)
                  and not (flags & _lib.GAGS_BWD_ATOMIC))
        ctx.geom_mfma = bool(geom_mfma and staged)
        ctx.save_for_backward(means2d, conics, colors, opacities, backgrounds, offsets, flatten_ids, packed, alphas,
                              last_ids, scratch if staged else None, blk_rows if staged else None)
        ctx.cfg = (width, height, flags)
        ctx.half = half
        ctx.rctx = rctx if rctx is not None else default_context()
        ctx.prezero = prezero if staged else None
        ctx.early = early if staged else None
        ctx.mark_non_differentiable(last_ids)
        return out, alphas, last_ids

    @staticmethod
    def backward(ctx, v_out, v_alphas, _v_last):
        lib = _lib.load()
        (means2d, conics, colors, opacities, backgrounds, offsets, flatten_ids, packed, alphas,
         last_ids, fwd_scratch, blk_rows) = ctx.saved_tensors
        width, height, flags = ctx.cfg
        n, d = colors.shape
        dev = colors.device
        n_isects = flatten_ids.shape[0]
        fwd = _FwdState(offsets, n_isects, blk_rows, fwd_scratch, flatten_ids, n, d, width, height)
        need_geom = ctx.needs_input_grad[0] or ctx.needs_input_grad[1] or ctx.needs_input_grad[3]
        v_out = torch.zeros(height, width, d, device=dev) if v_out is None else _c(v_out)
        v_alphas = None if v_alphas is None else _c(v_alphas)
        v_bg = None
        if backgrounds is not None and ctx.needs_input_grad[4]:
            v_bg = ((1.0 - alphas)[..., None] * v_out).sum(dim=(0, 1))
        if not need_geom and blk_rows is not None:
            v_colors = _backward_staged(lib, ctx.rctx, fwd, v_out, _stage_bits(flags, ctx.half), ctx.prezero, early=ctx.early)
            return None, None, v_colors, None, v_bg, None, None, None, None, None, None, None, None, None, None
        if need_geom and blk_rows is not None and ctx.geom_mfma:
            v_colors = None
            if ctx.needs_input_grad[2]:
                v_colors = _backward_staged(lib, ctx.rctx, fwd, v_out, _stage_bits(flags, ctx.half))
            if ctx.half:
                colors = colors.float()
            if GEOM_COMPACT_ROWS:
                incl = torch.cumsum(blk_rows, 0, dtype=torch.int32)
                row_base = (incl - blk_rows).contiguous()
                n_rows = int(incl[-1].item()) if incl.numel() else 0
            else:
                row_base, n_rows = None, -1
            nb = lib.gags_raster_bwd_geom_scratch_bytes(n_isects, width, height, n, d, n_rows)
            gscratch = torch.empty(nb, dtype=torch.uint8, device=dev)
            v_geo = torch.empty(n, 8, device=dev)
            with profiler.stage("raster_bwd_geom"):
                check(lib.gags_raster_bwd_geom(d, n, width, height, ptr(colors), ptr(backgrounds), ptr(offsets), n_isects,
                                               ptr(packed), ptr(v_out), ptr(v_alphas), ptr(blk_rows), ptr(fwd_scratch),
                                               fwd_scratch.numel(), ptr(gscratch), nb, ptr(v_geo), ptr(flatten_ids),
                                               ptr(row_base), n_rows,
                                               _lib.GAGS_RECS_BY_GAUSSIAN
                                               | (_lib.GAGS_GEOM_F32MFMA if (flags & _lib.GAGS_BWD_F32MFMA) else 0),
                                               _stream()),
                      "gags_raster_bwd_geom")
            v_con, v_m2d, v_opac = v_geo[:, 0:3].contiguous(), v_geo[:, 3:5].contiguous(), v_geo[:, 5].contiguous()
            return v_m2d, v_con, v_colors, v_opac, v_bg, None, None, None, None, None, None, None, None, None, None
        if ctx.half:
            colors = colors.float()
        v_colors = torch.zeros(n, d, device=dev)
        if need_geom:
            v_opac = torch.zeros(n, device=dev)
            v_m2d = torch.zeros(n, 2, device=dev)
            v_con = torch.zeros(n, 3, device=dev)
            bflags = (flags & 3) | _lib.GAGS_RECS_BY_GAUSSIAN
        else:
            v_opac = v_m2d = v_con = None
            bflags = (flags & 3) | _lib.GAGS_BWD_COLORS_ONLY | _lib.GAGS_RECS_BY_GAUSSIAN
        with profiler.stage("raster_bwd"):
            check(lib.gags_raster_bwd(d, width, height, ptr(means2d), ptr(conics), ptr(opacities), ptr(colors),
                                      ptr(backgrounds), ptr(offsets), ptr(flatten_ids), n_isects, ptr(packed),
                                      ptr(alphas), ptr(last_ids), ptr(v_out), ptr(v_alphas), ptr(v_colors),
                                      ptr(v_opac), ptr(v_m2d), ptr(v_con), bflags, _stream()), "gags_raster_bwd")
        if ctx.half:
            v_colors = v_colors.half()
        return v_m2d, v_con, v_colors, v_opac, v_bg, None, None, None, None, None, None, None, None, None, None


def _offsets_with_count(offsets, n_tiles, n_isects):
    if offsets.dim() == 1 and offsets.numel() == n_tiles + 1 and offsets.is_contiguous() and offsets.dtype == torch.int32:
        return offsets
    if offsets.numel() != n_tiles:
        raise ValueError(f"isect_offsets must have {n_tiles} (= tile_h * tile_w) entries, or {n_tiles + 1} with the count")
    full = torch.empty(n_tiles + 1, dtype=torch.int32, device=offsets.device)
    full[:n_tiles] = offsets.reshape(-1)
    full[n_tiles] = int(n_isects)
    return full


def _channel_ranges(d, spec):
    if isinstance(spec, int):
        if spec <= 0 or d % spec != 0 or d <= spec or spec % 32 != 0:
            return None
        return [(c, c + spec) for c in range(0, d, spec)]
    widths = [int(w) for w in spec]
    if not widths or any(w <= 0 or w % 128 != 0 for w in widths) or d % 128 != 0 or d <= widths[0]:
        return None
    out, c, i = [], 0, 0
    while c < d:
        w = min(widths[min(i, len(widths) - 1)], d - c)
        out.append((c, c + w))
        c, i = c + w, i + 1
    return out


def _geom_mfma_width(d):
    return d >= 16 and d % 8 == 0 and d <= 1024


class _EarlyRowmap:

    def __init__(self, trow, total, stmp, host, ev, rctx, dev):
        self.trow, self.total, self.stmp, self.host, self.ev, self.rctx, self.dev = trow, total, stmp, host, ev, rctx, dev
        self._rows = None

    def rows(self):
        if self._rows is None:
            self.ev.synchronize()
            self._rows = int(self.host[0])
            self.rctx.give_pinned(self.dev, self.host)
            self.host = None
        return self._rows

    def __del__(self):
        try:
            if self.host is not None:
                if self.ev.query():
                    self.rctx.give_pinned(self.dev, self.host)
                self.host = None
        except Exception:
            pass


class _FwdState(NamedTuple):
    offsets: Any
    n_isects: int
    blk_rows: Any
    fwd_scratch: Any
    flatten_ids: Any
    n: int
    d: int
    width: int
    height: int


_STAGE_NAMES = {_lib.GAGS_STAGE_ROWS: "bwd_rows", _lib.GAGS_STAGE_SORT: "bwd_sort", _lib.GAGS_STAGE_REDUCE: "bwd_reduce"}


def _stage_bits(raster_flags, half):
    return ((_lib.GAGS_STAGED_F32MFMA if (raster_flags & _lib.GAGS_BWD_F32MFMA) else 0)
            | (_lib.GAGS_STAGED_OUT_F16 if half else 0)
            | (_lib.GAGS_STAGED_BLOCKWAVES if (raster_flags & _lib.GAGS_BWD_BLOCKWAVES) else 0)
            | (_lib.GAGS_STAGED_EXACT_WEIGHTS if (raster_flags & _lib.GAGS_BWD_EXACT_WEIGHTS) else 0))


def _rowmap(lib, fwd):
    dev = fwd.blk_rows.device
    ne = lib.gags_bwd_rowmap_elems(fwd.n_isects, fwd.width, fwd.height)
    trow = torch.empty(ne, dtype=torch.int32, device=dev)
    total = torch.empty(1, dtype=torch.int32, device=dev)
    sb = lib.gags_bwd_rowmap_scratch_bytes(fwd.n_isects)
    stmp = torch.empty(max(sb, 4), dtype=torch.uint8, device=dev)
    check(lib.gags_bwd_rowmap(fwd.n_isects, fwd.width, fwd.height, ptr(fwd.offsets), ptr(fwd.blk_rows), ptr(fwd.fwd_scratch),
                              fwd.fwd_scratch.numel(), ptr(trow), ne, ptr(total), ptr(stmp), sb, _stream()), "gags_bwd_rowmap")
    return trow, total, stmp


def _early_rowmap(lib, rctx, fwd):
    trow, total, stmp = _rowmap(lib, fwd)
    dev = total.device
    host = rctx.take_pinned(dev)
    host.copy_(total, non_blocking=True)
    ev = torch.cuda.Event()
    ev.record()
    return _EarlyRowmap(trow, total, stmp, host, ev, rctx, dev)


def _row_count(lib, rctx, fwd, early, capacity):
    if early is not None:
        return early.trow, early.total, early.rows(), None
    with profiler.stage("bwd_rowcount"):
        trow, total, _ = _rowmap(lib, fwd)
        if capacity is not None:
            return trow, total, min(max(fwd.n_isects, 1), int(capacity * CAP_MARGIN) + 1024), _DeferredCount(total, rctx)
        host = ctypes.c_int32(0)
        check(lib.gags_read_i32(ptr(total), ctypes.byref(host), _stream()), "gags_read_i32")
        return trow, total, int(host.value), None


def _grad_buffer(rctx, fwd, bits, dev, hook, wire_hook, pending, prezero):
    v_dtype = torch.float16 if (bits & _lib.GAGS_STAGED_OUT_F16) else torch.float32
    if prezero is not None:
        buf, ev = prezero
        if hook is None and buf.shape == (fwd.n, fwd.d) and buf.dtype == v_dtype:
            torch.cuda.current_stream().wait_event(ev)
            return buf, None, bits | _lib.GAGS_STAGED_PREZEROED
    elif pending is None and (hook is None or (wire_hook is not None and rctx.grad_rows_hook is not None)):
        kept = rctx.kept_grad(fwd.n, fwd.d, v_dtype, dev)
        if kept is not None:
            return kept[0], kept, bits
    return torch.empty(fwd.n, fwd.d, device=dev, dtype=v_dtype), None, bits


def _bind_staged(lib, fwd, v_out, trow, rows, scratch, v_colors):
    fixed = (fwd.d, fwd.n, fwd.width, fwd.height, ptr(fwd.offsets), fwd.n_isects, ptr(v_out), ptr(fwd.blk_rows), ptr(trow), rows,
             ptr(fwd.fwd_scratch), fwd.fwd_scratch.numel(), ptr(scratch), scratch.numel(), ptr(v_colors))
    st = _stream()
    with_reduce = (_lib.GAGS_STAGE_ALL, _lib.GAGS_STAGE_REDUCE)

    def call(stage, c0, cw, rows_dev=None, wire=None, keep=None):
        if keep is not None and (stage & _lib.GAGS_STAGE_MASK) not in with_reduce:
            keep = None
        check(lib.gags_raster_bwd_colors_staged(
            *fixed, stage, c0, cw, rows_dev, ptr(wire[0]) if wire else None, ptr(wire[1]) if wire else None,
            ptr(keep[1]) if keep else None, ptr(keep[2]) if keep else None, st), "gags_raster_bwd_colors_staged")

    return call


def _run_whole(call, bits, d, rows_dev, kept, hook, v_colors):
    if profiler.ENABLED:
        for stage, name in _STAGE_NAMES.items():
            with profiler.stage(name):
                call(stage | bits, 0, d, rows_dev, None, kept)
    else:
        call(_lib.GAGS_STAGE_ALL | bits, 0, d, rows_dev, None, kept)
    if hook is not None:
        hook(v_colors.detach(), 0, d)


def _run_range_scratch(call, bits, d, kept):
    for c0 in range(0, d, 128):
        for stage in ((_lib.GAGS_STAGE_ROWS, _lib.GAGS_STAGE_SORT, _lib.GAGS_STAGE_REDUCE) if c0 == 0
                      else (_lib.GAGS_STAGE_ROWS, _lib.GAGS_STAGE_REDUCE)):
            with profiler.stage(_STAGE_NAMES[stage]):
                call(stage | bits | _lib.GAGS_STAGED_RANGE_SCRATCH, c0, 128, None, None, kept)


def _run_ranged(call, rctx, fwd, bits, ranges, hook, wire_hook, kept, v_colors):
    alias = v_colors.detach()
    group = max(int(rctx.grad_rows_group), 1)
    rows_done = 0
    for c0, c1 in ranges:
        if c1 > rows_done:
            g1 = rows_done
            while g1 < c1 or (g1 - rows_done < group and g1 < fwd.d):
                g1 = next(b for a, b in ranges if a == g1)
            for stage in ((_lib.GAGS_STAGE_ROWS, _lib.GAGS_STAGE_SORT) if rows_done == 0 else (_lib.GAGS_STAGE_ROWS,)):
                with profiler.stage(_STAGE_NAMES[stage]):
                    call(stage | bits, rows_done, g1 - rows_done)
            rows_done = g1
        w = wire_hook(c0, c1) if wire_hook is not None else None
        if w is None and kept is not None:
            rctx.forget_kept(fwd.n, fwd.d, v_colors.dtype, v_colors.device)
            kept = None
        with profiler.stage("bwd_reduce"):
            call(_lib.GAGS_STAGE_REDUCE | bits, c0, c1 - c0, None, w, kept)
        if w is not None:
            hook(alias, c0, c1, w[1])
        else:
            hook(alias, c0, c1)


def _backward_staged(lib, rctx, fwd, v_out, stage_bits=0, prezero=None, exact_rows=False, early=None):
    dev = v_out.device
    n, d = fwd.n, fwd.d
    hook = rctx.grad_range_hook
    if rctx.grad_rows_hook is not None and hook is not None:
        mask = torch.empty(n, dtype=torch.uint8, device=dev)
        check(lib.gags_blended_mask(fwd.n_isects, fwd.width, fwd.height, n, ptr(fwd.flatten_ids), ptr(fwd.fwd_scratch),
                                    fwd.fwd_scratch.numel(), ptr(mask), _stream()), "gags_blended_mask")
        rctx.grad_rows_hook(mask)
    ranges = _channel_ranges(d, rctx.grad_range_channels) if hook is not None else None
    cap_key = (n, fwd.width, fwd.height, dev.index)
    capacity = rctx.cap_rows.get(cap_key) if (rctx.capacity_mode and hook is None and not exact_rows) else None
    trow, total, rows, pending = _row_count(lib, rctx, fwd, early, capacity)
    narrow = (hook is None and pending is None and d % 128 == 0 and d > 128 and rows * d * 4 > PROW_MAX_BYTES)
    nbytes = lib.gags_bwd_staged_scratch_bytes(rows, n, 128 if narrow else d)
    scratch = torch.empty(nbytes, dtype=torch.uint8, device=dev)
    wire_hook = rctx.grad_wire_hook if (ranges is not None and not (stage_bits & _lib.GAGS_STAGED_OUT_F16)) else None
    v_colors, kept, bits = _grad_buffer(rctx, fwd, stage_bits, dev, hook, wire_hook, pending, prezero)
    call = _bind_staged(lib, fwd, v_out, trow, rows, scratch, v_colors)
    if narrow:
        _run_range_scratch(call, bits, d, kept)
    elif ranges is not None:
        _run_ranged(call, rctx, fwd, bits, ranges, hook, wire_hook, kept, v_colors)
    else:
        _run_whole(call, bits, d, ptr(total) if pending is not None else None, kept, hook, v_colors)
    if pending is not None:
        true_rows = pending.get()
        if true_rows > rows:
            rctx.cap_rows[cap_key] = true_rows
            return _backward_staged(lib, rctx, fwd, v_out, stage_bits, None, exact_rows=True)
        rows = true_rows
    if hook is None and rctx.capacity_mode:
        rctx.cap_rows[cap_key] = max(rows, int(0.97 * rctx.cap_rows.get(cap_key, 0)))
    profiler.note("bwd_rows", rows)
    return v_colors


def rasterization(means, quats, scales, opacities, colors, viewmats, Ks, width, height,
                  near_plane=0.01, far_plane=1e10, radius_clip=0.0, eps2d=0.3, sh_degree=None, packed=False,
                  tile_size=16, backgrounds=None, render_mode="RGB", sparse_grad=False, absgrad=False,
                  rasterize_mode="classic", channel_chunk=32, distributed=False, camera_model="pinhole",
                  covars=None, raster_flags=0, raw_params=False, scaling_modifier=1.0, context=None):
    rctx = context if context is not None else default_context()
    if tile_size != TILE:
        raise NotImplementedError("tile_size must be 16 (the gsplat default the reference relies on)")
    if rasterize_mode != "classic" or camera_model != "pinhole" or covars is not None or distributed or absgrad:
        raise NotImplementedError("only the options the reference uses are implemented "
                                  "(classic mode, pinhole camera, quats+scales)")
    if render_mode not in ("RGB", "D", "ED", "RGB+D", "RGB+ED"):
        raise ValueError(f"unknown render_mode {render_mode}")
    if viewmats.dim() != 3 or viewmats.shape[0] != 1 or Ks.shape[0] != 1:
        raise NotImplementedError("one camera per call (the reference renders one view per iteration, train.py:134-142)")
    n = means.shape[0]
    if means.shape != (n, 3) or quats.shape != (n, 4) or scales.shape != (n, 3):
        raise ValueError("means [N,3], quats [N,4], scales [N,3] expected")
    if opacities.shape != (n,) and not (raw_params and opacities.shape == (n, 1)):
        raise ValueError("opacities [N] expected" + (" (or the stored [N,1] logits with raw_params)" if raw_params else ""))
    _need_cuda(means, quats, scales, opacities, colors, viewmats, Ks, backgrounds)
    width, height = int(width), int(height)
    viewmat, K = viewmats[0], Ks[0]

    records = None
    if raw_params:
        dfinal = (3 if sh_degree is not None else colors.shape[-1]) + (1 if render_mode in ("RGB+D", "RGB+ED") else 0)
        if render_mode in ("D", "ED"):
            dfinal = 1
        radii, means2d, depths, conics, tiles, opacities, records = _ProjectRaw.apply(
            means, quats, scales, opacities, viewmat, K, width, height, float(eps2d), float(near_plane), float(far_plane),
            float(radius_clip), float(scaling_modifier), bool(_mfma_width(dfinal) and n > 0))
        if records.numel() == 0:
            records = None
    else:
        radii, means2d, depths, conics, tiles = _Project.apply(means, quats, scales, viewmat, K, width, height,
                                                               float(eps2d), float(near_plane), float(far_plane),
                                                               float(radius_clip))
    means2d_c = means2d[None]
    means2d = means2d_c[0]
    if sh_degree is not None:
        if colors.dim() != 3 or colors.shape[2] != 3:
            raise ValueError("SH colours must be [N,K,3]")
        campos = torch.inverse(viewmat.double())[:3, 3].float()
        cols = _SH.apply(colors, means, campos, radii, int(sh_degree))
    else:
        if colors.dim() != 2 or colors.shape[0] != n:
            raise ValueError("colors must be [N,D] when sh_degree is None")
        cols = colors
    bg = None if backgrounds is None else backgrounds.reshape(-1)
    if render_mode in ("RGB+D", "RGB+ED"):
        cols = torch.cat([cols, depths[:, None]], dim=-1)
        if bg is not None:
            bg = torch.cat([bg, torch.zeros(1, device=bg.device)])
    elif render_mode in ("D", "ED"):
        cols = depths[:, None]
        bg = None if bg is None else torch.zeros(1, device=bg.device)

    prezero = None
    dz = cols.shape[-1]
    if (rctx.overlap_zero_fill and rctx.grad_range_hook is None and torch.is_grad_enabled() and cols.requires_grad and _mfma_width(dz)
            and dz <= 1024 and n * dz >= ZERO_FILL_MIN_ELEMS and not (raster_flags & (_lib.GAGS_BWD_ATOMIC | _lib.GAGS_FWD_NO_MFMA
                                                                                      | _lib.GAGS_FWD_FUSED))
            and not (means.requires_grad or quats.requires_grad or scales.requires_grad or opacities.requires_grad)):
        vbuf = torch.empty(n, dz, device=cols.device, dtype=torch.float16 if cols.dtype == torch.float16 else torch.float32)
        side = rctx.side_stream(cols.device)
        ev0, ev1 = torch.cuda.Event(), torch.cuda.Event()
        ev0.record()
        with torch.cuda.stream(side):
            side.wait_event(ev0)
            vbuf.zero_()
            ev1.record()
        vbuf.record_stream(side)
        prezero = (vbuf, ev1)

    dcols = cols.shape[-1]
    wide = _mfma_width(dcols)
    cap_key = (n, width, height, means.device.index)

    def run(cap):
        with torch.no_grad(), profiler.stage("binning"):
            b = tile_binning(means2d, radii, depths, tiles, width, height, conics if wide else None,
                             _c(opacities) if wide else None, cap, records=records if wide else None, context=rctx)
        offs, flat = b.offsets_full, b.flatten_ids
        trimmed = None
        n_full = flat.shape[0]
        if (cap is None and wide and b.packed is not None and n_full > 0 and rctx.trim_lists is not False
                and not (raster_flags & (_lib.GAGS_FWD_NO_MFMA | _lib.GAGS_FWD_FUSED))):
            lib_ = _lib.load()
            if rctx.trim_lists or lib_.gags_raster_fwd_scratch_bytes(n_full, width, height) > TRIM_AUTO_BYTES:
                with torch.no_grad():
                    trimmed = _trim_lists(lib_, n, width, height, offs, flat, n_full, b.packed)
                offs, flat = trimmed[0], trimmed[1]
        r = _Rasterize.apply(means2d, conics, cols, opacities, bg, offs, flat, b.packed, width, height, int(raster_flags), prezero,
                             rctx, None, torch.is_grad_enabled())
        if trimmed is not None:
            with torch.no_grad():
                last_user = r[2].clone()
                check(_lib.load().gags_trim_last_ids(width, height, ptr(b.offsets_full), ptr(offs), ptr(r[1]), ptr(last_user), _stream()),
                      "gags_trim_last_ids")
            profiler.note("isects_trimmed", trimmed[2])
            r = (r[0], r[1], last_user, trimmed[2])
        else:
            r = (r[0], r[1], r[2], None)
        return b, r

    cap = None
    if rctx.capacity_mode and cap_key in rctx.cap_isects:
        cap = min(MAX_ISECTS - 1, int(rctx.cap_isects[cap_key] * CAP_MARGIN) + 4096)
    (isect_ids, flatten_ids, isect_offsets, n_isects, packed, _), (out, alphas, last_ids, n_trimmed) = run(cap)
    if cap is not None:
        n_true = n_isects.get()
        _check_isects(n_true, _tiles(width, height)[2])
        if n_true > cap:
            (isect_ids, flatten_ids, isect_offsets, n_isects, packed, _), (out, alphas, last_ids, n_trimmed) = run(None)
        else:
            n_isects = n_true
            isect_ids, flatten_ids = isect_ids[:n_true], flatten_ids[:n_true]
    if rctx.capacity_mode:
        rctx.cap_isects[cap_key] = max(n_isects, int(0.97 * rctx.cap_isects.get(cap_key, 0)))
    if render_mode in ("ED", "RGB+ED"):
        if out.requires_grad:
            out = torch.cat([out[..., :-1], out[..., -1:] / alphas[..., None].clamp(min=1e-10)], dim=-1)
        else:
            check(_lib.load().gags_ed_normalize(height * width, out.shape[-1], ptr(out), ptr(alphas), _stream()),
                  "gags_ed_normalize")

    tile_w, tile_h, _ = _tiles(width, height)
    info = {
        "camera_ids": None, "gaussian_ids": None,
        "radii": radii[None], "means2d": means2d_c, "depths": depths[None], "conics": conics[None],
        "opacities": opacities[None], "tile_width": tile_w, "tile_height": tile_h,
        "tiles_per_gauss": tiles[None], "isect_ids": isect_ids, "flatten_ids": flatten_ids,
        "isect_offsets": isect_offsets[None], "last_ids": last_ids, "width": width, "height": height,
        "tile_size": TILE, "n_cameras": 1, "n_isects": n_isects,
        "n_isects_trimmed": n_trimmed,
    }
    return out[None], alphas[None, ..., None], info
```

### include/gags_raster.h

```cpp
#ifndef GAGS_RASTER_H
#define GAGS_RASTER_H

#include <stdint.h>

#ifdef __cplusplus
extern "C" {
#endif
#pragma GCC visibility push(default)

#define GAGS_TILE 16
#define GAGS_MAX_ISECTS (1ll << 28)

#define GAGS_OK 0
#define GAGS_EINVAL (-1)
#define GAGS_ELAUNCH (-2)
#define GAGS_ESCRATCH (-3)
#define GAGS_ENODEV (-4)

#define GAGS_BWD_COLORS_ONLY 1
#define GAGS_FWD_NO_MFMA 2
#define GAGS_FEAT_F16 32
#define GAGS_FWD_F16MFMA 64

#define GAGS_FWD_EXACT 2048

#define GAGS_FWD_ONLY_WEIGHTS 512
#define GAGS_FWD_ONLY_FEATURES 1024

#define GAGS_RECS_BY_GAUSSIAN 256

int gags_abi_version(void);
const char *gags_strerror(int code);
int gags_device_count(void);

int gags_project_fwd(int n, const float *means, const float *quats, const float *scales,
                     const float *viewmat, const float *K, int width, int height,
                     float eps2d, float near_plane, float far_plane, float radius_clip,
                     int32_t *radii, float *means2d, float *depths, float *conics,
                     int32_t *tiles_per_gauss, void *stream);

int64_t gags_scan_scratch_bytes(int n);
int gags_cumsum_i32(int n, const int32_t *in, int32_t *cum, int32_t *total,
                    void *scratch, int64_t scratch_bytes, void *stream);

int gags_cumsum_gather_i32(int n, const int32_t *in, const int32_t *idx, int32_t *cum, int32_t *total,
                           void *scratch, int64_t scratch_bytes, void *stream);

int gags_read_i32(const int32_t *src, int32_t *dst_host, void *stream);

int64_t gags_depth_order_scratch_bytes(int n);
int gags_depth_order(int n, const float *depths, const int32_t *tiles_per_gauss, int32_t *order,
                     int32_t *tiles_ordered, void *scratch, int64_t scratch_bytes, void *stream);

int gags_tile_emit(int n, const float *means2d, const int32_t *radii, const float *depths,
                   const int32_t *cum, const int32_t *order, int tile_w, int tile_h,
                   int64_t *isect_ids, int32_t *flatten_ids, void *stream);

int gags_tile_emit_cap(int n, const float *means2d, const int32_t *radii, const float *depths, const int32_t *cum,
                       const int32_t *order, int tile_w, int tile_h, int64_t *isect_ids, int32_t *flatten_ids, int64_t cap,
                       const int32_t *total, void *stream);

int64_t gags_sort_scratch_bytes(int64_t n_isects);
int gags_sort_pairs(int64_t n_isects, int tile_bits, int depth_sorted,
                    const int64_t *keys_in, const int32_t *vals_in,
                    int64_t *keys_out, int32_t *vals_out,
                    void *scratch, int64_t scratch_bytes, void *stream);

int gags_tile_offsets(int64_t n_isects, const int64_t *sorted_ids, int n_tiles,
                      int32_t *isect_offsets, void *stream);

#define GAGS_PACKED_BYTES 32
int gags_pack_isects(int n, int64_t n_isects, const int32_t *flatten_ids, const float *means2d,
                     const float *conics, const float *opacities, const int32_t *radii, void *grec,
                     void *packed, void *stream);

int64_t gags_raster_fwd_scratch_bytes(int64_t n_isects, int width, int height);
int gags_raster_fwd(int d, int n, int width, int height, const float *means2d, const float *conics,
                    const float *opacities, const float *colors, const float *backgrounds,
                    const int32_t *isect_offsets, const int32_t *flatten_ids, int64_t n_isects,
                    const void *packed ,
                    float *render_colors, float *render_alphas, int32_t *last_ids,
                    void *scratch, int64_t scratch_bytes, int32_t *blk_rows,
                    int flags, void *stream);

int gags_raster_list_need(int n, int width, int height, const int32_t *isect_offsets, const int32_t *flatten_ids,
                          int64_t n_isects, const void *packed, int flags, int32_t *need, void *stream);
int gags_trim_lists(int width, int height, const int32_t *isect_offsets, const int32_t *need_cum,
                    const int32_t *flatten_ids, int32_t *offsets_out, int32_t *flatten_out, void *stream);
int gags_trim_last_ids(int width, int height, const int32_t *isect_offsets, const int32_t *offsets_trimmed,
                       const float *render_alphas, int32_t *last_ids, void *stream);

int gags_raster_bwd(int d, int width, int height, const float *means2d, const float *conics,
                    const float *opacities, const float *colors, const float *backgrounds,
                    const int32_t *isect_offsets, const int32_t *flatten_ids, int64_t n_isects,
                    const void *packed ,
                    const float *render_alphas, const int32_t *last_ids,
                    const float *v_render_colors, const float *v_render_alphas,
                    float *v_colors, float *v_opacities, float *v_means2d, float *v_conics,
                    int flags, void *stream);

int64_t gags_bwd_rowmap_elems(int64_t n_isects, int width, int height);
int64_t gags_bwd_rowmap_scratch_bytes(int64_t n_isects);
int gags_bwd_rowmap(int64_t n_isects, int width, int height, const int32_t *isect_offsets, const int32_t *blk_rows,
                    const void *fwd_scratch, int64_t fwd_scratch_bytes, int32_t *rowmap, int64_t rowmap_elems,
                    int32_t *total, void *scratch, int64_t scratch_bytes, void *stream);
#define GAGS_GEOM_F32MFMA 32
int64_t gags_raster_bwd_geom_scratch_bytes(int64_t n_isects, int width, int height, int n, int d, int64_t n_rows);
int gags_raster_bwd_geom(int d, int n, int width, int height, const float *colors, const float *backgrounds,
                         const int32_t *isect_offsets, int64_t n_isects, const void *packed,
                         const float *v_render_colors, const float *v_render_alphas, const int32_t *blk_rows,
                         const void *fwd_scratch, int64_t fwd_scratch_bytes, void *scratch, int64_t scratch_bytes,
                         float *v_geo, const int32_t *flatten_ids, const int32_t *row_base, int64_t n_rows, int flags,
                         void *stream);

int gags_blended_mask(int64_t n_isects, int width, int height, int n, const int32_t *flatten_ids,
                      const void *fwd_scratch, int64_t fwd_scratch_bytes, unsigned char *mask, void *stream);
#define GAGS_STAGE_ALL 0
#define GAGS_STAGE_ROWS 1
#define GAGS_STAGE_SORT 2
#define GAGS_STAGE_REDUCE 3
#define GAGS_STAGE_MASK 15
#define GAGS_STAGED_F32MFMA 32
#define GAGS_STAGED_OUT_F16 64
#define GAGS_STAGED_PREZEROED 128
#define GAGS_STAGED_RANGE_SCRATCH 256
#define GAGS_STAGED_BLOCKWAVES 512
#define GAGS_STAGED_EXACT_WEIGHTS 1024
int64_t gags_bwd_staged_scratch_bytes(int64_t rows, int n, int d);
int gags_raster_bwd_colors_staged(int d, int n, int width, int height, const int32_t *isect_offsets, int64_t n_isects,
                                  const float *v_render_colors, const int32_t *blk_rows, const int32_t *rowmap, int64_t rows,
                                  const void *fwd_scratch, int64_t fwd_scratch_bytes, void *scratch, int64_t scratch_bytes,
                                  float *v_colors, int stage, int ch_begin, int ch_count, const int32_t *rows_dev,
                                  const int32_t *wire_pos, float *wire, const uint8_t *keep_prev, uint8_t *keep_cur,
                                  void *stream);

int gags_raster_stats(int width, int height, const float *means2d, const float *conics,
                      const float *opacities, const int32_t *isect_offsets, const int32_t *flatten_ids,
                      int64_t n_isects, int64_t *counts, void *stream);

int gags_project_fwd_raw(int n, const float *means, const float *rotation, const float *scaling_log,
                         const float *opacity_logit, float scaling_modifier, const float *viewmat, const float *K,
                         int width, int height, float eps2d, float near_plane, float far_plane, float radius_clip,
                         int32_t *radii, float *means2d, float *depths, float *conics, int32_t *tiles_per_gauss,
                         float *opacities, float *quats_act, float *scales_act, void *grec, void *stream);
int gags_project_bwd_raw(int n, const float *means, const float *rotation, const float *scaling_log,
                         const float *opacity_logit, float scaling_modifier, const float *viewmat, const float *K,
                         int width, int height, float eps2d, const int32_t *radii, const float *v_means2d,
                         const float *v_depths, const float *v_conics, const float *v_opacities, float *v_means,
                         float *v_rotation, float *v_scaling_log, float *v_opacity_logit, void *stream);

int gags_project_bwd(int n, const float *means, const float *quats, const float *scales,
                     const float *viewmat, const float *K, int width, int height, float eps2d,
                     const int32_t *radii, const float *conics,
                     const float *v_means2d, const float *v_depths, const float *v_conics,
                     float *v_means, float *v_quats, float *v_scales, void *stream);

int gags_sh_fwd(int n, int kc, int degree, const float *means, const float *campos,
                const float *coeffs, const int32_t *radii, float *out, void *stream);
int gags_sh_bwd(int n, int kc, int degree, const float *means, const float *campos,
                const int32_t *radii, const float *colors_out, const float *v_out,
                float *v_coeffs, void *stream);

int gags_sh_bwd_dirs(int n, int kc, int degree, const float *means, const float *campos, const float *coeffs,
                     const int32_t *radii, const float *colors_out, const float *v_out, float *v_means, void *stream);

int gags_ed_normalize(int64_t n_pix, int d, float *render_colors, const float *render_alphas,
                      void *stream);

int gags_adam_step(int64_t numel, float *param, const float *grad, float *exp_avg, float *exp_avg_sq,
                   double lr, double beta1, double beta2, double eps, int step, void *stream);

int64_t gags_compact_mask_scratch_bytes(int n);
int gags_compact_mask(int n, const uint8_t *mask, int64_t cap, int64_t *idx, int32_t *count, void *scratch,
                      int64_t scratch_bytes, void *stream);
int gags_compact_mask_pos(int n, const uint8_t *mask, int64_t cap, int64_t *idx, int32_t *pos, int32_t *count, void *scratch,
                          int64_t scratch_bytes, void *stream);
int gags_pack_rows(int64_t n_rows, const int64_t *idx, const void *grad, int grad_type, int d, int c0, int cw,
                   void *wire, int wire_type, void *stream);
int gags_unpack_rows(int64_t n_rows, const int64_t *idx, const void *wire, int wire_type, const void *local,
                     void *grad, int grad_type, int d, int c0, int cw, void *stream);

int64_t gags_dot_scratch_bytes(void);
int gags_dot_f32(int64_t numel, const float *x, const float *y, float *out, void *scratch,
                 int64_t scratch_bytes, void *stream);

#pragma GCC visibility pop
#ifdef __cplusplus
}
#endif
#endif
```

Baseline: 127.2.

## Sort tile keys as 32-bit with stable radix and fuse scan spine

Tile binning now emits 32-bit tile-only keys, relying on the depth-ordered input plus a stable radix sort instead of sorting 64-bit tile|depth keys. Digits can be up to 11 bits wide, and the last pass rebuilds the 64-bit ids from the depths. Binning, sort and offset computation move into one entry point. The prefix scan drops its single-block spine kernel: each final block sums the preceding block totals itself, which saves a launch but repeats reads of the block sums.

```diff
diff --git a/gags_amd/_lib.py b/gags_amd/_lib.py
--- a/gags_amd/_lib.py
+++ b/gags_amd/_lib.py
@@ -31,6 +31,8 @@
     "gags_sort_scratch_bytes": (_i64, [_i64]),
     "gags_sort_pairs": (_i32, [_i64, _i32, _i32, _vp, _vp, _vp, _vp, _vp, _i64, _vp]),
     "gags_tile_offsets": (_i32, [_i64, _vp, _i32, _vp, _vp]),
+    "gags_bin_tiles_scratch_bytes": (_i64, [_i64]),
+    "gags_bin_tiles": (_i32, [_i32, _vp, _vp, _vp, _vp, _vp, _i32, _i32, _i64, _vp, _vp, _vp, _vp, _vp, _i64, _vp]),
     "gags_pack_isects": (_i32, [_i32, _i64, _vp, _vp, _vp, _vp, _vp, _vp, _vp, _vp]),
     "gags_raster_fwd_scratch_bytes": (_i64, [_i64, _i32, _i32]),
     "gags_raster_fwd": (_i32, [_i32, _i32, _i32, _i32, _vp, _vp, _vp, _vp, _vp, _vp, _vp, _i64, _vp, _vp, _vp, _vp,
diff --git a/gags_amd/csrc/api.hip b/gags_amd/csrc/api.hip
--- a/gags_amd/csrc/api.hip
+++ b/gags_amd/csrc/api.hip
@@ -246,11 +246,13 @@
     if (fwd_scratch_bytes < L.total) return GAGS_ESCRATCH;
     hipStream_t st = (hipStream_t)stream;
     int32_t *trow = rowmap;
-    if (hipMemsetAsync(trow, 0, sizeof(int32_t), st) != hipSuccess) return GAGS_ELAUNCH;
-    if (n_isects == 0) return hipMemsetAsync(total, 0, sizeof(int32_t), st) == hipSuccess ? GAGS_OK : GAGS_ELAUNCH;
+    if (n_isects == 0) {
+        if (hipMemsetAsync(trow, 0, sizeof(int32_t), st) != hipSuccess) return GAGS_ELAUNCH;
+        return hipMemsetAsync(total, 0, sizeof(int32_t), st) == hipSuccess ? GAGS_OK : GAGS_ELAUNCH;
+    }
     if (!scratch || scratch_bytes < gags_scan::scratch_bytes(n_isects)) return GAGS_ESCRATCH;
     const char *fs = (const char *)fwd_scratch;
-    gags_scan::launch<false>((int)n_isects, (const int32_t *)(fs + L.hit), trow + 1, total, (int32_t *)scratch, st);
+    gags_scan::launch<false>((int)n_isects, (const int32_t *)(fs + L.hit), trow + 1, total, (int32_t *)scratch, st, nullptr, trow);
     GAGS_CHECK_LAUNCH();
     return gags_bwd_slot_rows_launch(width, height, (int)n_isects, isect_offsets, blk_rows,
                                      (const int32_t *)(fs + L.sidx), trow, rowmap + rowmap_slot_off(n_isects), st);
diff --git a/gags_amd/csrc/binning.hip b/gags_amd/csrc/binning.hip
--- a/gags_amd/csrc/binning.hip
+++ b/gags_amd/csrc/binning.hip
@@ -1,16 +1,24 @@
+#include <type_traits>
+
 #include "common.h"
 #include "scan.h"
 
+int64_t gags_sort_tiles_scratch_bytes(int64_t n);
+int gags_sort_tiles(int64_t n, int nbits, uint32_t *keys, int32_t *vals, const uint32_t *low, uint32_t sentinel,
+                    uint64_t *ids_out, int32_t *vals_out, void *scratch, int64_t scratch_bytes, hipStream_t st);
+
 namespace {
 
+template <typename KT>
 __global__ __launch_bounds__(256) void tile_emit_kernel(int n, const float *__restrict__ means2d,
                                                         const int32_t *__restrict__ radii,
                                                         const float *__restrict__ depths,
                                                         const int32_t *__restrict__ cum,
                                                         const int32_t *__restrict__ order, int tile_w, int tile_h,
-                                                        int64_t *__restrict__ isect_ids,
+                                                        KT *__restrict__ isect_ids,
                                                         int32_t *__restrict__ flatten_ids, int64_t cap)
 {
+    constexpr bool WIDE = std::is_same<KT, int64_t>::value;
     __shared__ int s_rel[4][64], s_x0[4][64], s_y0[4][64], s_w[4][64], s_gid[4][64];
     __shared__ uint32_t s_dbits[4][64];
     const int lane = threadIdx.x & 63, w = threadIdx.x >> 6;
@@ -25,14 +33,15 @@
     if (rad > 0) {
         const float2 m = reinterpret_cast<const float2 *>(means2d)[i];
         gags_tile_aabb(m.x, m.y, rad, tile_w, tile_h, x0, x1, y0, y1);
-        dbits = (uint32_t)__float_as_int(depths[i]);
+        if (WIDE) dbits = (uint32_t)__float_as_int(depths[i]);
     }
     const int base = (jw == 0) ? 0 : cum[jw - 1];
     const int start = live ? ((j == 0) ? 0 : cum[j - 1]) : 0x7fffffff;
     const int jl = min(jw + 63, n - 1);
     const int total = cum[jl] - base;
     s_rel[w][lane] = live ? start - base : 0x7fffffff;
-    s_x0[w][lane] = x0; s_y0[w][lane] = y0; s_w[w][lane] = max(x1 - x0, 1); s_gid[w][lane] = i; s_dbits[w][lane] = dbits;
+    s_x0[w][lane] = x0; s_y0[w][lane] = y0; s_w[w][lane] = max(x1 - x0, 1); s_gid[w][lane] = i;
+    if (WIDE) s_dbits[w][lane] = dbits;
     __builtin_amdgcn_wave_barrier();
     for (int t = lane; t < total; t += 64) {
         int l = 0;
@@ -45,18 +54,20 @@
         const int64_t tile_id = (int64_t)(s_y0[w][l] + dy) * tile_w + (s_x0[w][l] + (r - dy * ww));
         const int64_t pos = (int64_t)base + t;
         if (pos < cap) {
-            isect_ids[pos] = (tile_id << 32) | (int64_t)s_dbits[w][l];
+            if constexpr (WIDE) isect_ids[pos] = (tile_id << 32) | (int64_t)s_dbits[w][l];
+            else isect_ids[pos] = (uint32_t)tile_id;
             flatten_ids[pos] = s_gid[w][l];
         }
     }
 }
 
+template <typename KT>
 __global__ __launch_bounds__(256) void isect_tail_kernel(int64_t cap, const int32_t *__restrict__ total, int n_tiles,
-                                                         int64_t *__restrict__ isect_ids, int32_t *__restrict__ flatten_ids)
+                                                         KT *__restrict__ isect_ids, int32_t *__restrict__ flatten_ids)
 {
     const int64_t i = (int64_t)blockIdx.x * 256 + threadIdx.x;
     if (i >= cap || i < (int64_t)total[0]) return;
-    isect_ids[i] = (int64_t)n_tiles << 32;
+    isect_ids[i] = std::is_same<KT, int64_t>::value ? (KT)((int64_t)n_tiles << 32) : (KT)n_tiles;
     flatten_ids[i] = 0;
 }
 
@@ -175,10 +186,10 @@
     if (!isect_ids || !flatten_ids || (n > 0 && (!means2d || !radii || !depths || !cum))) return GAGS_EINVAL;
     hipStream_t st = (hipStream_t)stream;
     if (n > 0)
-        hipLaunchKernelGGL(tile_emit_kernel, dim3((n + 255) / 256), dim3(256), 0, st, n, means2d, radii, depths, cum, order, tile_w,
+        hipLaunchKernelGGL(tile_emit_kernel<int64_t>, dim3((n + 255) / 256), dim3(256), 0, st, n, means2d, radii, depths, cum, order, tile_w,
                            tile_h, isect_ids, flatten_ids, cap);
     if (total && cap > 0)
-        hipLaunchKernelGGL(isect_tail_kernel, dim3((unsigned)((cap + 255) / 256)), dim3(256), 0, st, cap, total, tile_w * tile_h,
+        hipLaunchKernelGGL(isect_tail_kernel<int64_t>, dim3((unsigned)((cap + 255) / 256)), dim3(256), 0, st, cap, total, tile_w * tile_h,
                            isect_ids, flatten_ids);
     GAGS_CHECK_LAUNCH();
     return GAGS_OK;
@@ -207,6 +218,51 @@
     if (!sorted_ids) return GAGS_EINVAL;
     hipLaunchKernelGGL(tile_offsets_kernel, dim3((unsigned)((n_isects + 255) / 256)), dim3(256), 0, st, n_isects,
                        sorted_ids, n_tiles + 1, isect_offsets);
+    GAGS_CHECK_LAUNCH();
+    return GAGS_OK;
+}
+
+extern "C" int64_t gags_bin_tiles_scratch_bytes(int64_t size)
+{
+    const int64_t m = size > 0 ? size : 1;
+    return 2 * ((m * 4 + 255) / 256 * 256) + gags_sort_tiles_scratch_bytes(m);
+}
+
+extern "C" int gags_bin_tiles(int n, const float *means2d, const int32_t *radii, const float *depths, const int32_t *cum,
+                              const int32_t *order, int tile_w, int tile_h, int64_t size, const int32_t *total,
+                              int64_t *isect_ids, int32_t *flatten_ids, int32_t *isect_offsets, void *scratch,
+                              int64_t scratch_bytes, void *stream)
+{
+    GAGS_CLEAR_ERR();
+    if (n < 0 || tile_w <= 0 || tile_h <= 0 || size < 0 || size >= (1ll << 31) || (int64_t)tile_w * tile_h >= (1ll << 31) ||
+        !isect_offsets)
+        return GAGS_EINVAL;
+    const int n_tiles = tile_w * tile_h;
+    hipStream_t st = (hipStream_t)stream;
+    if (size == 0) {
+        hipLaunchKernelGGL(fill_i32_kernel, dim3((n_tiles + 1 + 255) / 256), dim3(256), 0, st, n_tiles + 1, 0, isect_offsets);
+        GAGS_CHECK_LAUNCH();
+        return GAGS_OK;
+    }
+    if (!isect_ids || !flatten_ids || !scratch || (n > 0 && (!means2d || !radii || !depths || !cum))) return GAGS_EINVAL;
+    if (n == 0 && !total) return GAGS_EINVAL;
+    if (scratch_bytes < gags_bin_tiles_scratch_bytes(size)) return GAGS_ESCRATCH;
+    const int64_t half = (size * 4 + 255) / 256 * 256;
+    uint32_t *keys = (uint32_t *)scratch;
+    int32_t *vals = (int32_t *)((char *)scratch + half);
+    if (n > 0)
+        hipLaunchKernelGGL(tile_emit_kernel<uint32_t>, dim3((n + 255) / 256), dim3(256), 0, st, n, means2d, radii, depths, cum, order,
+                           tile_w, tile_h, keys, vals, size);
+    if (total)
+        hipLaunchKernelGGL(isect_tail_kernel<uint32_t>, dim3((unsigned)((size + 255) / 256)), dim3(256), 0, st, size, total, n_tiles,
+                           keys, vals);
+    int tile_bits = 1;
+    while (tile_bits < 31 && (n_tiles >> tile_bits)) ++tile_bits;
+    const int rc = gags_sort_tiles(size, tile_bits, keys, vals, reinterpret_cast<const uint32_t *>(depths), (uint32_t)n_tiles,
+                                   (uint64_t *)isect_ids, flatten_ids, (char *)scratch + 2 * half, scratch_bytes - 2 * half, st);
+    if (rc != GAGS_OK) return rc;
+    hipLaunchKernelGGL(tile_offsets_kernel, dim3((unsigned)((size + 255) / 256)), dim3(256), 0, st, size, isect_ids, n_tiles + 1,
+                       isect_offsets);
     GAGS_CHECK_LAUNCH();
     return GAGS_OK;
 }
diff --git a/gags_amd/csrc/exchange.hip b/gags_amd/csrc/exchange.hip
--- a/gags_amd/csrc/exchange.hip
+++ b/gags_amd/csrc/exchange.hip
@@ -4,6 +4,31 @@
 #include "scan.h"
 
 namespace {
+
+__global__ __launch_bounds__(gags_scan::SCAN_THREADS) void scan_spine(int nb, int32_t *__restrict__ block_sums,
+                                                           int32_t *__restrict__ total_out)
+{
+    __shared__ int smem[4];
+    __shared__ double wide[gags_scan::SCAN_THREADS];
+    int carry = 0;
+    double dsum = 0.0;
+    for (int base = 0; base < nb; base += gags_scan::SCAN_THREADS) {
+        const int i = base + threadIdx.x;
+        const int v = (i < nb) ? block_sums[i] : 0;
+        dsum += (double)v;
+        int total;
+        const int incl = gags_scan::block_incl_scan(v, total, smem);
+        if (i < nb) block_sums[i] = carry + incl - v;
+        carry += total;
+    }
+    wide[threadIdx.x] = dsum;
+    __syncthreads();
+    if (threadIdx.x == 0 && total_out) {
+        double t = 0.0;
+        for (int k = 0; k < gags_scan::SCAN_THREADS; ++k) t += wide[k];
+        total_out[0] = (t > 2147483647.0) ? -1 : carry;
+    }
+}
 
 template <int T> struct Elem;
 template <> struct Elem<0> {
@@ -246,7 +271,7 @@
     const int nb = (n + CM_TILE - 1) / CM_TILE;
     int32_t *bs = (int32_t *)scratch;
     hipLaunchKernelGGL(cm_count_kernel, dim3(nb), dim3(256), 0, st, n, mask, bs);
-    hipLaunchKernelGGL(gags_scan::scan_spine, dim3(1), dim3(gags_scan::SCAN_THREADS), 0, st, nb, bs, count);
+    hipLaunchKernelGGL(scan_spine, dim3(1), dim3(gags_scan::SCAN_THREADS), 0, st, nb, bs, count);
     hipLaunchKernelGGL(cm_scatter_kernel, dim3(nb), dim3(256), 0, st, n, mask, bs, count, cap, idx, pos);
     GAGS_CHECK_LAUNCH();
     return GAGS_OK;
diff --git a/gags_amd/csrc/scan.h b/gags_amd/csrc/scan.h
--- a/gags_amd/csrc/scan.h
+++ b/gags_amd/csrc/scan.h
@@ -53,38 +53,39 @@
     if (threadIdx.x == 0) block_sums[blockIdx.x] = total;
 }
 
-__global__ __launch_bounds__(SCAN_THREADS) void scan_spine(int nb, int32_t *__restrict__ block_sums,
-                                                           int32_t *__restrict__ total_out)
+template <bool EXCLUSIVE>
+__global__ __launch_bounds__(SCAN_THREADS) void scan_final(int n, const int32_t *in ,
+                                                            const int32_t *__restrict__ idx,
+                                                            const int32_t *__restrict__ block_sums,
+                                                            int32_t *out, int32_t *__restrict__ total_out,
+                                                            int32_t *__restrict__ zero_word)
 {
     __shared__ int smem[4];
     __shared__ double wide[SCAN_THREADS];
-    int carry = 0;
-    double dsum = 0.0;
-    for (int base = 0; base < nb; base += SCAN_THREADS) {
-        const int i = base + threadIdx.x;
-        const int v = (i < nb) ? block_sums[i] : 0;
-        dsum += (double)v;
-        int total;
-        const int incl = block_incl_scan(v, total, smem);
-        if (i < nb) block_sums[i] = carry + incl - v;
-        carry += total;
+    const bool last = blockIdx.x == gridDim.x - 1;
+    if (zero_word && blockIdx.x == 0 && threadIdx.x == 0) zero_word[0] = 0;
+    const int lim = last ? (int)gridDim.x : (int)blockIdx.x;
+    uint32_t part = 0;
+    double dpart = 0.0;
+    for (int i = threadIdx.x; i < lim; i += SCAN_THREADS) {
+        const int b = block_sums[i];
+        part += (uint32_t)b;
+        dpart += (double)b;
     }
-    wide[threadIdx.x] = dsum;
-    __syncthreads();
-    if (threadIdx.x == 0 && total_out) {
-        double t = 0.0;
-        for (int k = 0; k < SCAN_THREADS; ++k) t += wide[k];
-        total_out[0] = (t > 2147483647.0) ? -1 : carry;
+    int before;
+    block_incl_scan((int)part, before, smem);
+    if (last) {
+        before = (int)((uint32_t)before - (uint32_t)block_sums[blockIdx.x]);
+        if (total_out) {
+            wide[threadIdx.x] = dpart;
+            __syncthreads();
+            if (threadIdx.x == 0) {
+                double t = 0.0;
+                for (int k = 0; k < SCAN_THREADS; ++k) t += wide[k];
+                total_out[0] = (t > 2147483647.0) ? -1 : (int)((uint32_t)before + (uint32_t)block_sums[blockIdx.x]);
+            }
+        }
     }
-}
-
-template <bool EXCLUSIVE>
-__global__ __launch_bounds__(SCAN_THREADS) void scan_final(int n, const int32_t *in ,
-                                                            const int32_t *__restrict__ idx,
-                                                            const int32_t *__restrict__ block_offs,
-                                                            int32_t *out)
-{
-    __shared__ int smem[4];
     const int base = blockIdx.x * SCAN_TILE + threadIdx.x * SCAN_ITEMS;
     int v[SCAN_ITEMS];
     int s = 0;
@@ -96,7 +97,7 @@
     }
     int total;
     const int incl = block_incl_scan(s, total, smem);
-    int run = block_offs[blockIdx.x] + incl - s;
+    int run = before + incl - s;
 #pragma unroll
     for (int k = 0; k < SCAN_ITEMS; ++k) {
         const int i = base + k;
@@ -121,12 +122,12 @@
 
 template <bool EXCLUSIVE>
 inline void launch(int n, const int32_t *in, int32_t *out, int32_t *total, int32_t *block_scratch, hipStream_t st,
-                   const int32_t *idx = nullptr)
+                   const int32_t *idx = nullptr, int32_t *zero_word = nullptr)
 {
     const int nb = (n + SCAN_TILE - 1) / SCAN_TILE;
     hipLaunchKernelGGL(scan_block_sums, dim3(nb), dim3(SCAN_THREADS), 0, st, n, in, idx, block_scratch);
-    hipLaunchKernelGGL(scan_spine, dim3(1), dim3(SCAN_THREADS), 0, st, nb, block_scratch, total);
-    hipLaunchKernelGGL(scan_final<EXCLUSIVE>, dim3(nb), dim3(SCAN_THREADS), 0, st, n, in, idx, block_scratch, out);
+    hipLaunchKernelGGL(scan_final<EXCLUSIVE>, dim3(nb), dim3(SCAN_THREADS), 0, st, n, in, idx, block_scratch, out, total,
+                       zero_word);
 }
 
 }
diff --git a/gags_amd/csrc/sort.hip b/gags_amd/csrc/sort.hip
--- a/gags_amd/csrc/sort.hip
+++ b/gags_amd/csrc/sort.hip
@@ -1,29 +1,48 @@
+#include <type_traits>
+
 #include "common.h"
 #include "scan.h"
 
+#ifndef GAGS_RS_MAX_DIGIT
+#define GAGS_RS_MAX_DIGIT 8
+#endif
+static_assert(GAGS_RS_MAX_DIGIT >= 1 && GAGS_RS_MAX_DIGIT <= 11, "digits of 1 to 11 bits");
+
 namespace {
 
 constexpr int RS_THREADS = 256;
-constexpr int RS_ITEMS = 8;
-constexpr int RS_TILE = RS_THREADS * RS_ITEMS;
-constexpr int RS_RADIX = 256;
-
-template <typename K>
-__global__ __launch_bounds__(RS_THREADS) void rs_histogram(int64_t n, int shift, const K *__restrict__ keys,
+constexpr int RS_MAX_DIGIT = GAGS_RS_MAX_DIGIT;
+constexpr int RSCAN_ITEMS = 8;
+constexpr int RSCAN_TILE = RS_THREADS * RSCAN_ITEMS;
+
+template <int RB>
+struct RsShape {
+    static constexpr int RADIX = 1 << RB;
+    static constexpr int ITEMS = RB <= 8 ? 8 : 16;
+    static constexpr int TILE = RS_THREADS * ITEMS;
+    static constexpr int PER = RADIX / RS_THREADS;
+    using Cnt = typename std::conditional<RB <= 8, uint32_t, uint16_t>::type;
+};
+
+template <typename K, int RB>
+__global__ __launch_bounds__(RS_THREADS) void rs_histogram(int64_t n, int shift, int bits, const K *__restrict__ keys,
                                                            uint32_t *__restrict__ hist ,
                                                            int nblocks)
 {
-    __shared__ uint32_t h[RS_RADIX];
-    h[threadIdx.x] = 0;
-    __syncthreads();
-    const int64_t base = (int64_t)blockIdx.x * RS_TILE;
-#pragma unroll
-    for (int k = 0; k < RS_ITEMS; ++k) {
+    using S = RsShape<RB>;
+    __shared__ uint32_t h[S::RADIX];
+    const int radix = 1 << bits;
+    const uint32_t mask = (uint32_t)radix - 1u;
+    for (int d = threadIdx.x; d < radix; d += RS_THREADS) h[d] = 0;
+    __syncthreads();
+    const int64_t base = (int64_t)blockIdx.x * S::TILE;
+#pragma unroll
+    for (int k = 0; k < S::ITEMS; ++k) {
         const int64_t i = base + k * RS_THREADS + threadIdx.x;
-        if (i < n) atomicAdd(&h[(keys[i] >> shift) & 0xff], 1u);
-    }
-    __syncthreads();
-    hist[(size_t)threadIdx.x * nblocks + blockIdx.x] = h[threadIdx.x];
+        if (i < n) atomicAdd(&h[(uint32_t)(keys[i] >> shift) & mask], 1u);
+    }
+    __syncthreads();
+    for (int d = threadIdx.x; d < radix; d += RS_THREADS) hist[(size_t)d * nblocks + blockIdx.x] = h[d];
 }
 
 __global__ __launch_bounds__(RS_THREADS) void rs_rowscan(int nblocks, uint32_t *__restrict__ hist, uint32_t *__restrict__ totals)
@@ -31,12 +50,12 @@
     __shared__ int smem[4];
     uint32_t *row = hist + (size_t)blockIdx.x * nblocks;
     uint32_t carry = 0;
-    for (int base = 0; base < nblocks; base += RS_TILE) {
-        const int i0 = base + threadIdx.x * RS_ITEMS;
-        uint32_t v[RS_ITEMS];
+    for (int base = 0; base < nblocks; base += RSCAN_TILE) {
+        const int i0 = base + threadIdx.x * RSCAN_ITEMS;
+        uint32_t v[RSCAN_ITEMS];
         uint32_t s = 0;
 #pragma unroll
-        for (int k = 0; k < RS_ITEMS; ++k) {
+        for (int k = 0; k < RSCAN_ITEMS; ++k) {
             v[k] = (i0 + k < nblocks) ? row[i0 + k] : 0u;
             s += v[k];
         }
@@ -44,7 +63,7 @@
         const int incl = gags_scan::block_incl_scan((int)s, total, smem);
         uint32_t run = carry + (uint32_t)incl - s;
 #pragma unroll
-        for (int k = 0; k < RS_ITEMS; ++k) {
+        for (int k = 0; k < RSCAN_ITEMS; ++k) {
             if (i0 + k < nblocks) row[i0 + k] = run;
             run += v[k];
         }
@@ -53,43 +72,64 @@
     if (threadIdx.x == 0) totals[blockIdx.x] = carry;
 }
 
-template <typename K>
-__global__ __launch_bounds__(RS_THREADS) void rs_scatter(int64_t n, int shift, const K *__restrict__ keys_in,
+template <typename K, typename KO, int RB>
+__global__ __launch_bounds__(RS_THREADS) void rs_scatter(int64_t n, int shift, int bits, const K *__restrict__ keys_in,
                                                          const int32_t *__restrict__ vals_in,
-                                                         K *__restrict__ keys_out,
+                                                         KO *__restrict__ keys_out,
                                                          int32_t *__restrict__ vals_out,
                                                          const uint32_t *__restrict__ hist, int nblocks,
-                                                         const uint32_t *__restrict__ totals)
-{
-    __shared__ uint32_t cnt_s[4][RS_RADIX];
-    volatile uint32_t(*cnt)[RS_RADIX] = cnt_s;
-    __shared__ uint32_t gbase[RS_RADIX];
+                                                         const uint32_t *__restrict__ totals,
+                                                         const uint32_t *__restrict__ low, uint32_t sentinel)
+{
+    using S = RsShape<RB>;
+    using Cnt = typename S::Cnt;
+    constexpr int ITEMS = S::ITEMS, TILE = S::TILE, PER = S::PER, RADIX = S::RADIX;
+    __shared__ Cnt cnt_s[4][RADIX];
+    volatile Cnt(*cnt)[RADIX] = cnt_s;
+    __shared__ uint32_t gbase[RADIX];
+    __shared__ Cnt dstart[RADIX];
     __shared__ int scan_tmp[4];
     const int lane = threadIdx.x & 63, w = threadIdx.x >> 6;
-#pragma unroll
-    for (int k = 0; k < 4; ++k) cnt[k][threadIdx.x] = 0;
+    const int radix = 1 << bits;
+    const uint32_t mask = (uint32_t)radix - 1u;
+    for (int d = threadIdx.x; d < radix; d += RS_THREADS) {
+#pragma unroll
+        for (int k = 0; k < 4; ++k) cnt[k][d] = 0;
+    }
     {
-        const uint32_t tot = totals[threadIdx.x];
+        uint32_t tot[PER];
+        uint32_t s = 0;
+#pragma unroll
+        for (int j = 0; j < PER; ++j) {
+            const int d = threadIdx.x * PER + j;
+            tot[j] = d < radix ? totals[d] : 0u;
+            s += tot[j];
+        }
         int all;
-        const int incl = gags_scan::block_incl_scan((int)tot, all, scan_tmp);
-        gbase[threadIdx.x] = ((uint32_t)incl - tot) + hist[(size_t)threadIdx.x * nblocks + blockIdx.x];
-    }
-    __syncthreads();
-
-    const int64_t wbase = (int64_t)blockIdx.x * RS_TILE + (int64_t)w * (64 * RS_ITEMS);
-    K key[RS_ITEMS];
-    int32_t val[RS_ITEMS];
-    uint32_t rank[RS_ITEMS];
-#pragma unroll
-    for (int k = 0; k < RS_ITEMS; ++k) {
+        const int incl = gags_scan::block_incl_scan((int)s, all, scan_tmp);
+        uint32_t run = (uint32_t)incl - s;
+#pragma unroll
+        for (int j = 0; j < PER; ++j) {
+            const int d = threadIdx.x * PER + j;
+            if (d < radix) gbase[d] = run + hist[(size_t)d * nblocks + blockIdx.x];
+            run += tot[j];
+        }
+    }
+    __syncthreads();
+
+    const int64_t wbase = (int64_t)blockIdx.x * TILE + (int64_t)w * (64 * ITEMS);
+    K key[ITEMS];
+    int32_t val[ITEMS];
+    uint32_t rank[ITEMS];
+#pragma unroll
+    for (int k = 0; k < ITEMS; ++k) {
         const int64_t i = wbase + k * 64 + lane;
         const bool ok = i < n;
         key[k] = ok ? keys_in[i] : (K)~(K)0;
         val[k] = ok ? (vals_in ? vals_in[i] : (int32_t)i) : 0;
-        const uint32_t dgt = ok ? (uint32_t)((key[k] >> shift) & 0xff) : 0xffffffffu;
+        const uint32_t dgt = ok ? ((uint32_t)(key[k] >> shift) & mask) : 0xffffffffu;
         uint64_t m = __ballot(ok);
-#pragma unroll
-        for (int b = 0; b < 8; ++b) {
+        for (int b = 0; b < bits; ++b) {
             const uint64_t bal = __ballot((dgt >> b) & 1u);
             m &= ((dgt >> b) & 1u) ? bal : ~bal;
         }
@@ -100,62 +140,117 @@
             prev = cnt[w][dgt];
         }
         __builtin_amdgcn_wave_barrier();
-        if (ok && lower == 0) cnt[w][dgt] = prev + (uint32_t)__popcll(m);
+        if (ok && lower == 0) cnt[w][dgt] = (Cnt)(prev + (uint32_t)__popcll(m));
         __builtin_amdgcn_wave_barrier();
         rank[k] = prev + before;
     }
     __syncthreads();
-    __shared__ uint32_t dstart[RS_RADIX];
     {
-        const int d = threadIdx.x;
-        uint32_t run = 0;
-#pragma unroll
-        for (int k = 0; k < 4; ++k) {
-            const uint32_t c = cnt[k][d];
-            cnt[k][d] = run;
-            run += c;
+        uint32_t dtot[PER];
+        uint32_t s = 0;
+#pragma unroll
+        for (int j = 0; j < PER; ++j) {
+            const int d = threadIdx.x * PER + j;
+            uint32_t run = 0;
+            if (d < radix) {
+#pragma unroll
+                for (int k = 0; k < 4; ++k) {
+                    const uint32_t c = cnt[k][d];
+                    cnt[k][d] = (Cnt)run;
+                    run += c;
+                }
+            }
+            dtot[j] = run;
+            s += run;
         }
         int total;
-        const int incl = gags_scan::block_incl_scan((int)run, total, scan_tmp);
-        dstart[d] = (uint32_t)incl - run;
-    }
-    __syncthreads();
-    __shared__ K keys_l[RS_TILE];
-    __shared__ int32_t vals_l[RS_TILE];
-#pragma unroll
-    for (int k = 0; k < RS_ITEMS; ++k) {
+        const int incl = gags_scan::block_incl_scan((int)s, total, scan_tmp);
+        uint32_t run = (uint32_t)incl - s;
+#pragma unroll
+        for (int j = 0; j < PER; ++j) {
+            const int d = threadIdx.x * PER + j;
+            if (d < radix) dstart[d] = (Cnt)run;
+            run += dtot[j];
+        }
+    }
+    __syncthreads();
+    __shared__ K keys_l[TILE];
+    __shared__ int32_t vals_l[TILE];
+#pragma unroll
+    for (int k = 0; k < ITEMS; ++k) {
         const int64_t i = wbase + k * 64 + lane;
         if (i < n) {
-            const uint32_t dgt = (uint32_t)((key[k] >> shift) & 0xff);
+            const uint32_t dgt = (uint32_t)(key[k] >> shift) & mask;
             const uint32_t lp = dstart[dgt] + cnt[w][dgt] + rank[k];
             keys_l[lp] = key[k];
             vals_l[lp] = val[k];
         }
     }
     __syncthreads();
-    const int64_t bbase = (int64_t)blockIdx.x * RS_TILE;
-    const int nvalid = (int)((n - bbase) < (int64_t)RS_TILE ? (n - bbase) : (int64_t)RS_TILE);
-#pragma unroll
-    for (int k = 0; k < RS_ITEMS; ++k) {
+    const int64_t bbase = (int64_t)blockIdx.x * TILE;
+    const int nvalid = (int)((n - bbase) < (int64_t)TILE ? (n - bbase) : (int64_t)TILE);
+#pragma unroll
+    for (int k = 0; k < ITEMS; ++k) {
         const int i = k * RS_THREADS + threadIdx.x;
         if (i < nvalid) {
             const K kk = keys_l[i];
-            const uint32_t dgt = (uint32_t)((kk >> shift) & 0xff);
+            const int32_t vv = vals_l[i];
+            const uint32_t dgt = (uint32_t)(kk >> shift) & mask;
             const uint32_t pos = gbase[dgt] + ((uint32_t)i - dstart[dgt]);
-            keys_out[pos] = kk;
-            vals_out[pos] = vals_l[i];
-        }
-    }
+            if constexpr (std::is_same<K, KO>::value) {
+                keys_out[pos] = kk;
+            } else {
+                const uint32_t lo = ((uint32_t)kk == sentinel) ? 0u : low[vv];
+                keys_out[pos] = ((KO)kk << 32) | (KO)lo;
+            }
+            vals_out[pos] = vv;
+        }
+    }
+}
+
+inline int64_t rs_al256(int64_t x) { return (x + 255) / 256 * 256; }
+
+struct RsPlan {
+    int passes, lo, rem;
+    explicit RsPlan(int nbits) : passes((nbits + RS_MAX_DIGIT - 1) / RS_MAX_DIGIT), lo(nbits / passes), rem(nbits % passes) {}
+    int bits(int p) const { return lo + (p < rem ? 1 : 0); }
+    int shift(int p) const { return p * lo + (p < rem ? p : rem); }
+    int max_bits() const { return lo + (rem ? 1 : 0); }
+};
+
+inline int64_t rs_hist_elems(int64_t n)
+{
+    const int64_t narrow = ((n + RsShape<8>::TILE - 1) / RsShape<8>::TILE) * RsShape<8>::RADIX;
+    const int64_t wide = RS_MAX_DIGIT > 8 ? ((n + RsShape<11>::TILE - 1) / RsShape<11>::TILE) * RsShape<11>::RADIX : 0;
+    return narrow > wide ? narrow : wide;
 }
 
 template <typename K>
 int64_t sort_scratch_bytes_t(int64_t n_in)
 {
     const int64_t n = n_in > 0 ? n_in : 1;
-    const int64_t nblocks = (n + RS_TILE - 1) / RS_TILE;
-    const int64_t keys = ((n * (int64_t)sizeof(K) + 255) / 256) * 256, vals = ((n * 4 + 255) / 256) * 256;
-    const int64_t hist = ((nblocks * RS_RADIX * 4 + 255) / 256) * 256;
-    return keys + vals + hist + RS_RADIX * 4;
+    return rs_al256(n * (int64_t)sizeof(K)) + rs_al256(n * 4) + rs_al256(rs_hist_elems(n) * 4) + (1 << RS_MAX_DIGIT) * 4;
+}
+
+template <typename K, typename KO, int RB>
+void rs_pass(int64_t n, int shift, int bits, const K *src_k, const int32_t *src_v, KO *dst_k, int32_t *dst_v, uint32_t *hist,
+             uint32_t *totals, const uint32_t *low, uint32_t sentinel, hipStream_t st)
+{
+    const int nblocks = (int)((n + RsShape<RB>::TILE - 1) / RsShape<RB>::TILE);
+    hipLaunchKernelGGL((rs_histogram<K, RB>), dim3(nblocks), dim3(RS_THREADS), 0, st, n, shift, bits, src_k, hist, nblocks);
+    hipLaunchKernelGGL(rs_rowscan, dim3(1 << bits), dim3(RS_THREADS), 0, st, nblocks, hist, totals);
+    hipLaunchKernelGGL((rs_scatter<K, KO, RB>), dim3(nblocks), dim3(RS_THREADS), 0, st, n, shift, bits, src_k, src_v, dst_k, dst_v,
+                       hist, nblocks, totals, low, sentinel);
+}
+
+template <typename K, typename KO>
+void rs_pass_any(int64_t n, int shift, int bits, const K *src_k, const int32_t *src_v, KO *dst_k, int32_t *dst_v, uint32_t *hist,
+                 uint32_t *totals, const uint32_t *low, uint32_t sentinel, hipStream_t st)
+{
+#if GAGS_RS_MAX_DIGIT > 8
+    if (bits > 8) return rs_pass<K, KO, 11>(n, shift, bits, src_k, src_v, dst_k, dst_v, hist, totals, low, sentinel, st);
+#endif
+    rs_pass<K, KO, 8>(n, shift, bits, src_k, src_v, dst_k, dst_v, hist, totals, low, sentinel, st);
 }
 
 template <typename K>
@@ -167,24 +262,19 @@
         return GAGS_EINVAL;
     if (!keys_in || !keys_out || !vals_out || !scratch) return GAGS_EINVAL;
     if (scratch_bytes < sort_scratch_bytes_t<K>(n)) return GAGS_ESCRATCH;
-    const int nblocks = (int)((n + RS_TILE - 1) / RS_TILE);
-    const int64_t keys_b = ((n * (int64_t)sizeof(K) + 255) / 256) * 256, vals_b = ((n * 4 + 255) / 256) * 256;
+    const int64_t keys_b = rs_al256(n * (int64_t)sizeof(K)), vals_b = rs_al256(n * 4);
     K *ktmp = (K *)scratch;
     int32_t *vtmp = (int32_t *)((char *)scratch + keys_b);
     uint32_t *hist = (uint32_t *)((char *)scratch + keys_b + vals_b);
-    const int64_t hist_b = (((int64_t)nblocks * RS_RADIX * 4 + 255) / 256) * 256;
-    uint32_t *totals = (uint32_t *)((char *)scratch + keys_b + vals_b + hist_b);
-    const int passes = (nbits + 7) / 8;
+    uint32_t *totals = (uint32_t *)((char *)scratch + keys_b + vals_b + rs_al256(rs_hist_elems(n) * 4));
+    const RsPlan plan(nbits);
     const K *src_k = keys_in;
     const int32_t *src_v = vals_in;
-    for (int p = 0; p < passes; ++p) {
-        const bool to_out = ((passes - 1 - p) % 2) == 0;
+    for (int p = 0; p < plan.passes; ++p) {
+        const bool to_out = ((plan.passes - 1 - p) % 2) == 0;
         K *dst_k = to_out ? keys_out : ktmp;
         int32_t *dst_v = to_out ? vals_out : vtmp;
-        hipLaunchKernelGGL(rs_histogram<K>, dim3(nblocks), dim3(RS_THREADS), 0, st, n, first_bit + p * 8, src_k, hist, nblocks);
-        hipLaunchKernelGGL(rs_rowscan, dim3(RS_RADIX), dim3(RS_THREADS), 0, st, nblocks, hist, totals);
-        hipLaunchKernelGGL(rs_scatter<K>, dim3(nblocks), dim3(RS_THREADS), 0, st, n, first_bit + p * 8, src_k, src_v, dst_k, dst_v,
-                           hist, nblocks, totals);
+        rs_pass_any<K, K>(n, first_bit + plan.shift(p), plan.bits(p), src_k, src_v, dst_k, dst_v, hist, totals, nullptr, 0u, st);
         src_k = dst_k;
         src_v = dst_v;
     }
@@ -192,6 +282,34 @@
     return GAGS_OK;
 }
 
+}
+
+int64_t gags_sort_tiles_scratch_bytes(int64_t n_in)
+{
+    const int64_t n = n_in > 0 ? n_in : 1;
+    return 2 * rs_al256(n * 4) + rs_al256(rs_hist_elems(n) * 4) + (1 << RS_MAX_DIGIT) * 4;
+}
+int gags_sort_tiles(int64_t n, int nbits, uint32_t *keys, int32_t *vals, const uint32_t *low, uint32_t sentinel,
+                    uint64_t *ids_out, int32_t *vals_out, void *scratch, int64_t scratch_bytes, hipStream_t st)
+{
+    if (n == 0) return GAGS_OK;
+    if (n < 0 || n >= (1ll << 31) || nbits <= 0 || nbits > 32 || !keys || !vals || !ids_out || !vals_out || !scratch)
+        return GAGS_EINVAL;
+    if (scratch_bytes < gags_sort_tiles_scratch_bytes(n)) return GAGS_ESCRATCH;
+    uint32_t *kb[2] = {keys, (uint32_t *)scratch};
+    int32_t *vb[2] = {vals, (int32_t *)((char *)scratch + rs_al256(n * 4))};
+    uint32_t *hist = (uint32_t *)((char *)scratch + 2 * rs_al256(n * 4));
+    uint32_t *totals = (uint32_t *)((char *)scratch + 2 * rs_al256(n * 4) + rs_al256(rs_hist_elems(n) * 4));
+    const RsPlan plan(nbits);
+    int cur = 0;
+    for (int p = 0; p + 1 < plan.passes; ++p, cur ^= 1)
+        rs_pass_any<uint32_t, uint32_t>(n, plan.shift(p), plan.bits(p), kb[cur], vb[cur], kb[cur ^ 1], vb[cur ^ 1], hist, totals,
+                                        nullptr, 0u, st);
+    const int p = plan.passes - 1;
+    rs_pass_any<uint32_t, uint64_t>(n, plan.shift(p), plan.bits(p), kb[cur], vb[cur], ids_out, vals_out, hist, totals, low, sentinel,
+                                    st);
+    GAGS_CHECK_LAUNCH();
+    return GAGS_OK;
 }
 
 int64_t gags_sort_u32_scratch_bytes(int64_t n) { return sort_scratch_bytes_t<uint32_t>(n); }
diff --git a/gags_amd/rasterization.py b/gags_amd/rasterization.py
--- a/gags_amd/rasterization.py
+++ b/gags_amd/rasterization.py
@@ -349,7 +349,6 @@
     dev = means2d.device
     n = radii.shape[0]
     tile_w, tile_h, n_tiles = _tiles(width, height)
-    tile_bits = max(1, n_tiles.bit_length())
     cum = torch.empty(max(n, 1), dtype=torch.int32, device=dev)
     total = torch.empty(1, dtype=torch.int32, device=dev)
     early = None
@@ -379,19 +378,13 @@
     else:
         size, count = int(cap), _DeferredCount(total, context or default_context())
     offsets = torch.empty(n_tiles + 1, dtype=torch.int32, device=dev)
-    ids = torch.empty(max(size, 1), dtype=torch.int64, device=dev)
-    flat = torch.empty(max(size, 1), dtype=torch.int32, device=dev)
-    ids_s = torch.empty_like(ids)
-    flat_s = torch.empty_like(flat)
-    if size > 0:
-        check(lib.gags_tile_emit_cap(n, ptr(means2d), ptr(radii), ptr(depths), ptr(cum), ptr(order), tile_w, tile_h,
-                                     ptr(ids), ptr(flat), size, ptr(total) if cap is not None else None, st),
-              "gags_tile_emit_cap")
-        ssb = lib.gags_sort_scratch_bytes(size)
-        sscratch = torch.empty(ssb, dtype=torch.uint8, device=dev)
-        check(lib.gags_sort_pairs(size, tile_bits, 1, ptr(ids), ptr(flat), ptr(ids_s), ptr(flat_s), ptr(sscratch),
-                                  ssb, st), "gags_sort_pairs")
-    check(lib.gags_tile_offsets(size, ptr(ids_s), n_tiles, ptr(offsets), st), "gags_tile_offsets")
+    ids_s = torch.empty(max(size, 1), dtype=torch.int64, device=dev)
+    flat_s = torch.empty(max(size, 1), dtype=torch.int32, device=dev)
+    bsb = lib.gags_bin_tiles_scratch_bytes(size)
+    bscratch = torch.empty(bsb, dtype=torch.uint8, device=dev)
+    check(lib.gags_bin_tiles(n, ptr(means2d), ptr(radii), ptr(depths), ptr(cum), ptr(order), tile_w, tile_h, size,
+                             ptr(total) if cap is not None else None, ptr(ids_s), ptr(flat_s), ptr(offsets), ptr(bscratch),
+                             bsb, st), "gags_bin_tiles")
     packed = records
     if conics is not None and packed is None:
         packed = torch.empty(max(n, 1), 8, dtype=torch.float32, device=dev)
diff --git a/include/gags_raster.h b/include/gags_raster.h
--- a/include/gags_raster.h
+++ b/include/gags_raster.h
@@ -68,6 +68,12 @@
 
 int gags_tile_offsets(int64_t n_isects, const int64_t *sorted_ids, int n_tiles,
                       int32_t *isect_offsets, void *stream);
+
+int64_t gags_bin_tiles_scratch_bytes(int64_t size);
+int gags_bin_tiles(int n, const float *means2d, const int32_t *radii, const float *depths, const int32_t *cum,
+                   const int32_t *order, int tile_w, int tile_h, int64_t size, const int32_t *total,
+                   int64_t *isect_ids, int32_t *flatten_ids, int32_t *isect_offsets,
+                   void *scratch, int64_t scratch_bytes, void *stream);
 
 #define GAGS_PACKED_BYTES 32
 int gags_pack_isects(int n, int64_t n_isects, const int32_t *flatten_ids, const float *means2d,
```

Measured after the change: 128.0, median of 6. About the same (+0.6%).
